# vganapati/CT_PVAE

Hardware: AMD Instinct MI355X
Metric: projections/sec (fwd+adj) 128x128 foam, 20 angles; fraction of HBM roofline (higher is better)
Workload: dtype f32; 1 GPU; batch=50/GPU 128x128 foam, 20 angles, P=184, rotate nearest fwd + tf_compat adj; objects_per_gpu=50, n_pixel=128, angles=20, num_proj_pix=184, parallelism=batch-shard x1, forward_plan=u16 taps, launch=19 replays of a HIP graph of 100 steps + 66 steps launched from Python

## Files before the change

ct_pvae_amd/_lib.py:

```python
import ctypes
import os

_HERE = os.path.dirname(os.path.abspath(__file__))
LIB_PATH = os.path.join(_HERE, "libctpvae_radon.so")

NEAREST, BILINEAR = 0, 1
NOISE = {"gaussian": 0, "poisson": 1}
BWD_TF_COMPAT, BWD_EXACT = 0, 1
SIDDON_STORE = {"raysum": 0, "sirt": 1, "tv_dual": 2, "gaussian": 3, "poisson": 4, "ratio": 5}
EINVAL, EHIP, ENODEV = -1, -2, -3
ABI_VERSION = 3400

_c_int, _c_float, _vp = ctypes.c_int, ctypes.c_float, ctypes.c_void_p
_ip = ctypes.POINTER(ctypes.c_int)

SIGNATURES = {
    "ctpvae_abi_version": (_c_int, []),
    "ctpvae_last_error": (ctypes.c_char_p, []),
    "ctpvae_device_count": (_c_int, []),
    "ctpvae_tune_set": (_c_int, [ctypes.c_char_p, _c_int]),
    "ctpvae_tune_active": (_c_int, []),
    "ctpvae_num_proj_pix": (_c_int, [_c_int, _c_int]),
    "ctpvae_pad_amounts": (_c_int, [_c_int, _c_int, _ip, _ip]),
    "ctpvae_rotate_transforms_f32": (_c_int, [_vp, _c_int, _c_int, _c_int, _vp, _vp, _vp]),
    "ctpvae_rotate_transforms_host_f32": (_c_int, [_vp, _c_int, _c_int, _c_int, _vp, _vp]),
    "ctpvae_rotate_fwd_planned_sel_f32": (_c_int, [_vp, _c_int, _c_int, _c_int, _c_int, _c_int, _c_int, _vp, _vp, _c_int, _vp, _vp]),
    "ctpvae_rotate_fwd_planned_loglik_sel_f32": (_c_int, [_vp, _c_int, _c_int, _c_int, _c_int, _c_int, _c_int, _vp, _vp, _c_int,
                                                          _vp, _vp, _c_int, _vp, _c_float, _vp, _vp, _vp, _vp]),
    "ctpvae_rotate_cplan_supported": (_c_int, [_c_int, _c_int, _c_int, _c_int, _c_int, _c_int]),
    "ctpvae_rotate_cplan_bytes": (ctypes.c_longlong, [_c_int, _c_int, _c_int, _c_int, _c_int]),
    "ctpvae_rotate_cplan_build_f32": (_c_int, [_vp, _c_int, _c_int, _c_int, _c_int, _c_int, _c_int, _c_int, _vp, _vp]),
    "ctpvae_rotate_cplan_overflowed": (_c_int, [_vp, _c_int, _c_int, _c_int, _c_int, _c_int, _vp]),
    "ctpvae_rotate_fwd_compact_f32": (_c_int, [_vp, _c_int, _c_int, _c_int, _c_int, _c_int, _c_int, _vp, _vp, _c_int, _c_int, _vp,
                                               _vp, _c_int, _vp, _c_float, _vp, _vp, _vp, _vp, _vp, _vp]),
    "ctpvae_rotate_fwd_compact_noise_f32": (_c_int, [_vp, _c_int, _c_int, _c_int, _c_int, _c_int, _c_int, _vp, _vp, _c_int, _c_int, _vp,
                                                     _vp, _c_int, _vp, _c_float, _c_int, _vp, _vp, _vp, _vp, _vp, _vp]),
    "ctpvae_loglik_tasks_per_row": (_c_int, [_c_int, _c_int]),
    "ctpvae_loglik_part_floats": (ctypes.c_longlong, [_c_int, _c_int, _c_int, _c_int]),
    "ctpvae_loglik_object_sums_f32": (_c_int, [_vp, _c_int, _c_int, _c_int, _c_int, _vp, _vp]),
    "ctpvae_rotate_bwd_sel_scaled_f32": (_c_int, [_vp, _c_int, _c_int, _c_int, _c_int, _vp, _vp, _c_int, _c_int, _c_int, _c_int,
                                                  _c_int, _vp, ctypes.c_longlong, _vp, _vp]),
    "ctpvae_rotate_bwd4_plan_bytes": (ctypes.c_longlong, [_c_int, _c_int, _c_int, _c_int, _c_int]),
    "ctpvae_rotate_bwd4_plan_build_f32": (_c_int, [_vp, _c_int, _c_int, _c_int, _c_int, _c_int, _c_int, _c_int, _vp, _vp]),
    "ctpvae_rotate_bwd_planned_sel_scaled_f32": (_c_int, [_vp, _c_int, _c_int, _c_int, _c_int, _c_int, _c_int, _vp, _vp, _c_int,
                                                          _c_int, _vp, ctypes.c_longlong, _vp, _vp]),
    "ctpvae_rotate_fwd_f32": (_c_int, [_vp, _c_int, _c_int, _c_int, _c_int, _c_int, _c_int, _c_int, _vp, _c_int,
                                       _c_int, _vp, _vp]),
    "ctpvae_rotate_fwd_f64": (_c_int, [_vp, _c_int, _c_int, _c_int, _c_int, _c_int, _c_int, _c_int, _vp, _c_int,
                                       _c_int, _vp, _vp]),
    "ctpvae_rotate_bwd_f64": (_c_int, [_vp, _c_int, _c_int, _c_int, _c_int, _vp, _c_int, _c_int, _c_int, _c_int,
                                       _c_int, _c_int, _vp, _vp]),
    "ctpvae_rotate_tile_shape": (_c_int, [_c_int, _c_int, _c_int, ctypes.POINTER(ctypes.c_int), ctypes.POINTER(ctypes.c_int)]),
    "ctpvae_rotate_fwd_tiled_workspace_bytes": (ctypes.c_longlong, [_c_int, _c_int, _c_int, _c_int, _c_int, _c_int, _c_int]),
    "ctpvae_rotate_fwd_tiled_f32": (_c_int, [_vp, _c_int, _c_int, _c_int, _c_int, _c_int, _c_int, _c_int, _vp, _c_int, _vp,
                                             _vp, _vp]),
    "ctpvae_rotate_fwd_tiled_interp_f32": (_c_int, [_vp, _c_int, _c_int, _c_int, _c_int, _c_int, _c_int, _c_int, _vp, _c_int, _c_int,
                                                    _vp, _vp, _vp]),
    "ctpvae_rotate_fwd_fast_f32": (_c_int, [_vp, _c_int, _c_int, _c_int, _c_int, _c_int, _c_int, _c_int, _vp, _c_int, _vp, _vp]),
    "ctpvae_rotate_fwd_tiled_fast_f32": (_c_int, [_vp, _c_int, _c_int, _c_int, _c_int, _c_int, _c_int, _c_int, _vp, _c_int, _vp,
                                                  _vp, _vp]),
    "ctpvae_rotate_fwd_tiled_loglik_f32": (_c_int, [_vp, _c_int, _c_int, _c_int, _c_int, _c_int, _c_int, _c_int, _vp, _c_int,
                                                    _vp, _vp, _vp, _vp, _c_float, _vp, _vp, _vp, _vp]),
    "ctpvae_rotate_tplan_bytes": (ctypes.c_longlong, [_c_int, _c_int, _c_int, _c_int, _c_int]),
    "ctpvae_rotate_tplan_build_f32": (_c_int, [_vp, _c_int, _c_int, _c_int, _c_int, _c_int, _c_int, _c_int, _vp, _vp]),
    "ctpvae_rotate_tplan_overflowed": (_c_int, [_vp, _c_int, _c_int, _c_int, _c_int, _c_int, _vp]),
    "ctpvae_rotate_fwd_tiled_compact_f32": (_c_int, [_vp, _c_int, _c_int, _c_int, _c_int, _c_int, _c_int, _c_int, _vp, _c_int, _vp,
                                                     _vp, _vp, _vp, _vp, _c_float, _vp, _vp, _vp, _vp, _vp, _vp]),
    "ctpvae_rotate_bwd_f32": (_c_int, [_vp, _c_int, _c_int, _c_int, _c_int, _vp, _c_int, _c_int, _c_int, _c_int,
                                       _c_int, _c_int, _vp, _vp]),
    "ctpvae_rotate_bwd_scaled_f32": (_c_int, [_vp, _c_int, _c_int, _c_int, _c_int, _vp, _c_int, _c_int, _c_int, _c_int,
                                              _c_int, _c_int, _vp, ctypes.c_longlong, _vp, _vp]),
    "ctpvae_rotate_plan_supported": (_c_int, [_c_int, _c_int, _c_int, _c_int, _c_int, _c_int, _c_int]),
    "ctpvae_rotate_plan_bytes": (ctypes.c_longlong, [_c_int, _c_int, _c_int, _c_int, _c_int, _c_int]),
    "ctpvae_rotate_plan_build_f32": (_c_int, [_vp, _vp, _c_int, _c_int, _c_int, _c_int, _c_int, _c_int, _c_int, _vp, _vp,
                                              _vp]),
    "ctpvae_rotate_fwd_planned_f32": (_c_int, [_vp, _c_int, _c_int, _c_int, _c_int, _c_int, _c_int, _vp, _vp, _vp]),
    "ctpvae_rotate_fwd_planned_form": (_c_int, [_c_int, _c_int, _c_int, _c_int, _c_int, _c_int, _c_int]),
    "ctpvae_rotate_fwd_planned_loglik_f32": (_c_int, [_vp, _c_int, _c_int, _c_int, _c_int, _c_int, _c_int, _vp, _vp, _vp, _vp,
                                                      _c_float, _vp, _vp, _vp, _vp]),
    "ctpvae_rotate_bwd_planned_f32": (_c_int, [_vp, _c_int, _c_int, _c_int, _c_int, _c_int, _c_int, _vp, _vp, _vp]),
    "ctpvae_rotate_bwd_planned_scaled_f32": (_c_int, [_vp, _c_int, _c_int, _c_int, _c_int, _c_int, _c_int, _vp, _vp,
                                                      ctypes.c_longlong, _vp, _vp]),
    "ctpvae_rotate_exact_plan_bytes": (ctypes.c_longlong, [_c_int, _c_int, _c_int, _c_int, _c_int]),
    "ctpvae_rotate_exact_plan_build_f32": (_c_int, [_vp, _vp, _c_int, _c_int, _c_int, _c_int, _c_int, _c_int, _c_int, _vp, _vp]),
    "ctpvae_rotate_exact_plan_overflowed": (_c_int, [_vp, _c_int, _c_int, _c_int, _c_int, _c_int, _vp]),
    "ctpvae_rotate_bwd_exact_planned_f32": (_c_int, [_vp, _c_int, _c_int, _c_int, _c_int, _c_int, _c_int, _vp, _vp, _vp]),
    "ctpvae_rotate_exact_wplan_bytes": (ctypes.c_longlong, [_c_int, _c_int, _c_int]),
    "ctpvae_rotate_exact_wplan_build_f32": (_c_int, [_vp, _vp, _c_int, _c_int, _c_int, _c_int, _c_int, _c_int, _c_int, _c_int, _vp, _vp]),
    "ctpvae_rotate_exact_wplan_overflowed": (_c_int, [_vp, _c_int, _c_int, _c_int, _vp]),
    "ctpvae_rotate_bwd_exact_wplan_f32": (_c_int, [_vp, _c_int, _c_int, _c_int, _c_int, _vp, _c_int, _c_int, _c_int, _c_int, _vp,
                                                              _vp, _vp]),
    "ctpvae_rotate_bwd_step_plan_bytes": (ctypes.c_longlong, [_c_int, _c_int, _c_int]),
    "ctpvae_rotate_bwd_step_plan_build_f32": (_c_int, [_vp, _c_int, _c_int, _c_int, _c_int, _c_int, _c_int, _c_int, _vp, _vp]),
    "ctpvae_rotate_bwd_step_plan_overflowed": (_c_int, [_vp, _c_int, _c_int, _c_int, _vp]),
    "ctpvae_rotate_bwd_stepped_scaled_f32": (_c_int, [_vp, _c_int, _c_int, _c_int, _c_int, _vp, _c_int, _c_int, _c_int, _c_int, _vp, _vp,
                                                      ctypes.c_longlong, _vp, _vp]),
    "ctpvae_siddon_dx": (_c_int, [_c_int, _c_int, _c_int]),
    "ctpvae_siddon_tables_f32": (_c_int, [_vp, _c_int, _vp, _vp, _vp]),
    "ctpvae_siddon_fwd_f32": (_c_int, [_vp, _c_int, _c_int, _c_int, _vp, _vp, _vp, _c_int, _c_int, _c_float, _vp,
                                       _vp]),
    "ctpvae_siddon_bwd_workspace_bytes": (ctypes.c_longlong, [_c_int, _c_int, _c_int, _c_int, _c_int]),
    "ctpvae_siddon_bwd_prepare_f32": (_c_int, [_c_int, _c_int, _vp, _vp, _vp, _c_int, _c_int, _c_float, _vp, _vp]),
    "ctpvae_siddon_bwd_prepared_f32": (_c_int, [_vp, _c_int, _c_int, _c_int, _vp, _vp, _vp, _c_int, _c_int, _c_float, _vp, _vp, _vp,
                                                _vp]),
    "ctpvae_siddon_fwd_workspace_bytes": (ctypes.c_longlong, [_c_int, _c_int, _c_int]),
    "ctpvae_siddon_fwd_ws_f32": (_c_int, [_vp, _c_int, _c_int, _c_int, _vp, _vp, _vp, _c_int, _c_int, _c_float, _vp, _vp, _vp, _vp,
                                          _vp]),
    "ctpvae_siddon_fwd_ws_tv_dual_f32": (_c_int, [_vp, _c_int, _c_int, _c_int, _vp, _vp, _vp, _c_int, _c_int, _c_float, _vp, _vp, _vp,
                                                  _vp, _vp]),
    "ctpvae_siddon_bwd_tv_primal_f32": (_c_int, [_vp, _c_int, _c_int, _c_int, _vp, _vp, _vp, _c_int, _c_int, _c_float, _vp, _vp,
                                                 _c_float, _vp, _vp, _vp, _vp, _vp, _vp, _vp, _vp]),
    "ctpvae_siddon_fwd_loglik_f32": (_c_int, [_vp, _c_int, _c_int, _c_int, _vp, _vp, _vp, _c_int, _c_int, _c_float, _vp, _c_int, _vp, _vp,
                                              _c_int, _vp, _c_float, _vp, _vp, _vp, _vp, _vp]),
    "ctpvae_siddon_fwd_loglik_noise_f32": (_c_int, [_vp, _c_int, _c_int, _c_int, _vp, _vp, _vp, _c_int, _c_int, _c_float, _vp, _c_int, _vp,
                                                    _vp, _c_int, _vp, _c_float, _c_int, _vp, _vp, _vp, _vp, _vp]),
    "ctpvae_siddon_bwd_sel_scaled_f32": (_c_int, [_vp, _c_int, _c_int, _c_int, _vp, _vp, _vp, _c_int, _c_int, _c_float, _vp, _c_int, _vp,
                                                  _vp, ctypes.c_longlong, _vp, _vp]),
    "ctpvae_siddon_fwd_ratio_f32": (_c_int, [_vp, _c_int, _c_int, _c_int, _vp, _vp, _vp, _c_int, _c_int, _c_float, _vp, _c_int, _vp, _vp,
                                             _vp, _vp]),
    "ctpvae_siddon_bwd_sel_mul_f32": (_c_int, [_vp, _c_int, _c_int, _c_int, _vp, _vp, _vp, _c_int, _c_int, _c_float, _vp, _c_int, _vp,
                                               _vp, _vp, _vp]),
    "ctpvae_siddon_bwd_sel_pml_f32": (_c_int, [_vp, _c_int, _c_int, _c_int, _vp, _vp, _vp, _c_int, _c_int, _c_float, _vp, _c_int, _vp,
                                               _vp, _c_float, _c_float, _c_int, _vp, _vp, _vp]),
    "ctpvae_siddon_fwd_resid_f32": (_c_int, [_vp, _c_int, _c_int, _c_int, _vp, _vp, _vp, _c_int, _c_int, _c_float, _vp, _vp, _vp,
                                             _vp]),
    "ctpvae_siddon_bwd_f32": (_c_int, [_vp, _c_int, _c_int, _c_int, _vp, _vp, _vp, _c_int, _c_int, _c_float, _vp, _vp, _vp]),
    "ctpvae_siddon_rownorm_f32": (_c_int, [_c_int, _c_int, _vp, _vp, _vp, _c_int, _c_int, _c_float, _vp, _vp]),
    "ctpvae_siddon_fwd_form": (_c_int, [_c_int, _c_int, _c_int, _c_int, _c_int, _c_int]),
    "ctpvae_fbp_filter_f64": (_c_int, [_vp, _c_int, _c_int, _vp, _vp, _vp]),
    "ctpvae_fbp_backproject_f64": (_c_int, [_vp, _c_int, _c_int, _c_int, _vp, _vp, _c_int, _c_int, _vp, _vp]),
    "ctpvae_fbp_backproject_bwd_f64": (_c_int, [_vp, _c_int, _c_int, _c_int, _vp, _vp, _c_int, _c_int, ctypes.c_double,
                                                ctypes.c_double, ctypes.c_double, _vp, _vp]),
    "ctpvae_fbp_backproject_geom_f64": (_c_int, [_vp, _c_int, _c_int, _c_int, _vp, _vp, _c_int, _c_int, ctypes.c_double,
                                                 ctypes.c_double, ctypes.c_double, _vp, _vp]),
    "ctpvae_gridrec_tables_bytes": (ctypes.c_longlong, [_c_int, _c_int]),
    "ctpvae_gridrec_tables_host_f32": (_c_int, [_c_int, _c_int, _c_float, _vp, _c_int, _vp, _vp]),
    "ctpvae_gridrec_workspace_bytes": (ctypes.c_longlong, [_c_int, _c_int, _c_int]),
    "ctpvae_gridrec_f32": (_c_int, [_vp, _c_int, _c_int, _c_int, _vp, _c_int, _c_int, _vp, _vp, _vp]),
    "ctpvae_poisson_loglik_fwd_f32": (_c_int, [_vp, _vp, _vp, _c_int, _c_int, _c_int, _vp, _vp, _vp]),
    "ctpvae_poisson_loglik_bwd_f32": (_c_int, [_vp, _vp, _vp, _vp, _c_int, _c_int, _c_int, _vp, _vp, _vp]),
    "ctpvae_loglik_fwd_f32": (_c_int, [_vp, _vp, _vp, _c_int, _c_int, _c_int, _vp, _c_float, _vp, _vp]),
    "ctpvae_poisson_measure_f32": (_c_int, [_vp, _vp, _c_int, _c_int, _c_int, _c_float, ctypes.c_ulonglong, _vp, _vp]),
    "ctpvae_philox4x32_10": (_c_int, [_vp, _vp, _vp]),
    "ctpvae_loglik_bwd_f32": (_c_int, [_vp, _vp, _vp, _vp, _c_int, _c_int, _c_int, _vp, _c_float, _vp, _vp, _vp]),
    "ctpvae_hmc_state_floats": (_c_int, [_c_int]),
    "ctpvae_hmc_init_f32": (_c_int, [_vp, _c_int, _c_int, _c_int, _vp, _vp, _c_int, _vp, _vp, _c_float, _c_int, _vp, _vp, _vp, _vp,
                                     _c_float, _vp]),
    "ctpvae_hmc_run_f32": (_c_int, [_vp, _c_int, ctypes.c_uint, _c_int, _c_int, _vp, _vp, _c_int, _vp, _vp, _c_float, _c_int, _vp, _vp,
                                    _vp, _c_int, _c_int, ctypes.c_uint, ctypes.c_uint, ctypes.c_ulonglong, _vp, _vp, _vp, _vp, _vp]),
    "ctpvae_tn_head_fwd_f32": (_c_int, [_vp, _vp, _c_int, _c_int, ctypes.c_longlong, ctypes.c_ulonglong, ctypes.c_uint, _vp, _vp, _vp, _vp,
                                        _vp]),
    "ctpvae_tn_head_bwd_f32": (_c_int, [_vp, _vp, _c_int, _c_int, ctypes.c_longlong, ctypes.c_ulonglong, ctypes.c_uint, _vp, _vp, _vp, _vp,
                                        _vp, _vp]),
    "ctpvae_tn_head_uniforms_host_f32": (_c_int, [_c_int, _c_int, ctypes.c_longlong, ctypes.c_ulonglong, ctypes.c_uint, _vp]),
    "ctpvae_tn_marginals_workspace_bytes": (ctypes.c_longlong, [_c_int, _c_int, ctypes.c_uint]),
    "ctpvae_tn_marginals_f32": (_c_int, [_vp, _vp, _c_int, _c_int, ctypes.c_longlong, ctypes.c_ulonglong, ctypes.c_uint, ctypes.c_uint,
                                         _c_float, _c_float, _c_int, _vp, _vp, _vp, _vp, _vp]),
    "ctpvae_tn_marginals_bin_host_f32": (_c_int, [_vp, ctypes.c_longlong, _c_float, _c_float, _c_int, _vp]),
    "ctpvae_latent_fwd_f32": (_c_int, [_vp, _c_int, _c_int, _c_int, _c_float, ctypes.c_longlong, ctypes.c_ulonglong, ctypes.c_uint,
                                       ctypes.c_uint, _vp, _vp, _vp, _vp, _vp, _vp]),
# ... 162 lines not shown
```

ct_pvae_amd/csrc/common.h:

```cpp
#pragma once
#include <hip/hip_runtime.h>
#include <atomic>
#include <cstdarg>
#include <cstdio>
#include <cstdlib>

#include "../../include/ctpvae_radon.h"

namespace ctpvae {

char *err_buf();
int fail(int code, const char *fmt, ...);

#define CTPVAE_REQUIRE(cond, ...)                                   \
    do {                                                            \
        if (!(cond)) return ::ctpvae::fail(CTPVAE_EINVAL, __VA_ARGS__); \
    } while (0)

#define CTPVAE_HIP(call)                                                                      \
    do {                                                                                      \
        hipError_t e_ = (call);                                                               \
        if (e_ != hipSuccess)                                                                 \
            return ::ctpvae::fail(CTPVAE_EHIP, "%s failed: %s", #call, hipGetErrorString(e_)); \
    } while (0)

#define CTPVAE_LAUNCH_CHECK(name)                                                             \
    do {                                                                                      \
        hipError_t e_ = hipGetLastError();                                                    \
        if (e_ != hipSuccess)                                                                 \
            return ::ctpvae::fail(CTPVAE_EHIP, "launch of %s failed: %s", name, hipGetErrorString(e_)); \
    } while (0)

constexpr int kMaxLdsBytes = 160 * 1024;

struct SliceScale {
    const float *ptr;
    long long stride;
    __device__ __forceinline__ float at(int s) const { return ptr ? ptr[(long long)s * stride] : 1.0f; }
};

enum StorePolicy { kStorePlain = 0, kStoreWriteThrough = 1, kStoreNonTemporal = 2 };
template <int ST> __device__ __forceinline__ void store_f32(float v, float *p)
{
    if constexpr (ST == kStoreWriteThrough) __hip_atomic_store(p, v, __ATOMIC_RELAXED, __HIP_MEMORY_SCOPE_AGENT);
    else if constexpr (ST == kStoreNonTemporal) __builtin_nontemporal_store(v, p);
    else *p = v;
}
template <int ST> __device__ __forceinline__ void store_f32x2(float v0, float v1, float *p)
{
    typedef float f2_t __attribute__((ext_vector_type(2)));
    const f2_t v = {v0, v1};
    if constexpr (ST == kStoreWriteThrough)
        __hip_atomic_store(reinterpret_cast<unsigned long long *>(p), __builtin_bit_cast(unsigned long long, v), __ATOMIC_RELAXED,
                           __HIP_MEMORY_SCOPE_AGENT);
    else if constexpr (ST == kStoreNonTemporal) __builtin_nontemporal_store(v, reinterpret_cast<f2_t *>(p));
    else *reinterpret_cast<f2_t *>(p) = v;
}

#define CTPVAE_SET_MAX_LDS_ONCE(kernel, seen)                                                                     \
    do {                                                                                                          \
        int dev_ = 0;                                                                                             \
        CTPVAE_HIP(hipGetDevice(&dev_));                                                                          \
        const unsigned long long bit_ = 1ull << (dev_ & 63);                                                      \
        if (dev_ >= 64 || !((seen).load(std::memory_order_acquire) & bit_)) {                                     \
            CTPVAE_HIP(hipFuncSetAttribute((const void *)(kernel), hipFuncAttributeMaxDynamicSharedMemorySize,    \
                                           ::ctpvae::kMaxLdsBytes));                                              \
            if (dev_ < 64) (seen).fetch_or(bit_, std::memory_order_release);                                      \
        }                                                                                                         \
    } while (0)

#define CTPVAE_REQUIRE_NO_STATIC_LDS(kernel, name, seen)                                                           \
    do {                                                                                                          \
        int dev_ = 0;                                                                                             \
        CTPVAE_HIP(hipGetDevice(&dev_));                                                                          \
        const unsigned long long bit_ = 1ull << (dev_ & 63);                                                      \
        const int fake_ = ::ctpvae::knob(::ctpvae::kKnobFakeStaticLds);                                            \
        if (dev_ >= 64 || fake_ > 0 || !((seen).load(std::memory_order_acquire) & bit_)) {                        \
            hipFuncAttributes fa_;                                                                                \
            CTPVAE_HIP(hipFuncGetAttributes(&fa_, (const void *)(kernel)));                                       \
            const long long static_ = (long long)fa_.sharedSizeBytes + (fake_ > 0 ? fake_ : 0);                    \
            if (static_ != 0)                                                                                     \
                return ::ctpvae::fail(CTPVAE_EHIP, "%s was built with %lld bytes of static LDS: its gathers address LDS " \
                                      "absolutely and need the dynamic array at address 0 -- rebuild the library (no "    \
                                      "__shared__ variables in these kernels)", name, static_);                   \
            if (dev_ < 64 && fake_ <= 0) (seen).fetch_or(bit_, std::memory_order_release);                        \
        }                                                                                                         \
    } while (0)

enum Knob {
    kKnobNoPlan, kKnobForceGeneric, kKnobNs, kKnobG, kKnobWaves, kKnobBns, kKnobBw, kKnobSegNs, kKnobSegChunk,
    kKnobSegPpt, kKnobTiledNs, kKnobTiledG, kKnobSiddonNs, kKnobSiddonThreads, kKnobSiddonPpb, kKnobMaxSlices,
    kKnobSiddonBwdNs, kKnobSiddonBwdChunks, kKnobNoCompact, kKnobSkew0, kKnobTiledSort, kKnobTiledPair, kKnobAffine, kKnobFakeStaticLds, kKnobFoldSums, kKnobTiledXcd, kKnobTiledWaves, kKnobTiledTh, kKnobReduceWaves, kKnobStepNs, kKnobStepLdsKb, kKnobTiledForce, kKnobBsort, kKnobMixG, kKnobMixG2, kKnobMixU1, kKnobNoMagic, kKnobMixG1, kKnobMixG3, kKnobMixU2, kKnobBrsplit, kKnobFwdFew, kKnobWtStores, kKnobBwdTail, kKnobCount
};
int knob(Knob k);

inline int store_policy(int rule)
{
    const int v = knob(kKnobWtStores);
    return v >= 0 && v <= 2 ? v : rule;
}

inline int max_slices_per_launch()
{
    const int v = knob(kKnobMaxSlices);
    return (v >= 1 && v <= 65535) ? v : 65535;
}

inline int ceil_div(int a, int b) { return (a + b - 1) / b; }

}
```

ct_pvae_amd/csrc/core.hip:

```cpp
#include <cmath>
#include <cstring>

#include "common.h"

namespace ctpvae {

char *err_buf()
{
    static thread_local char buf[512] = {0};
    return buf;
}

int fail(int code, const char *fmt, ...)
{
    va_list ap;
    va_start(ap, fmt);
    vsnprintf(err_buf(), 512, fmt, ap);
    va_end(ap);
    return code;
}

static const char *const kKnobNames[kKnobCount] = {
    "NO_PLAN", "FORCE_GENERIC", "NS", "G", "WAVES", "BNS", "BW", "SEG_NS", "SEG_CHUNK", "SEG_PPT", "TILED_NS", "TILED_G",
    "SIDDON_NS", "SIDDON_THREADS", "SIDDON_PPB", "MAX_SLICES", "SIDDON_BWD_NS", "SIDDON_BWD_CHUNKS", "NO_COMPACT", "SKEW0", "TILED_SORT", "TILED_PAIR", "AFFINE", "FAKE_STATIC_LDS", "FOLD_SUMS", "TILED_XCD", "TILED_WAVES", "TILED_TH", "REDUCE_WAVES", "STEP_NS", "STEP_LDS_KB", "TILED_FORCE", "BSORT", "MIXG", "MIXG_G2", "MIXG_U1", "NO_MAGIC", "MIXG_G1", "MIXG_G3", "MIXG_U2", "BRSPLIT", "FWD_FEW", "WT_STORES", "BWD_TAIL"};
static std::atomic<int> g_knobs[kKnobCount];
static int find_knob(const char *name)
{
    for (int k = 0; k < kKnobCount; ++k)
        if (strcmp(name, kKnobNames[k]) == 0) return k;
    return -1;
}
static const bool g_knobs_loaded = [] {
    for (int k = 0; k < kKnobCount; ++k) {
        int v = -1;
        char env[64];
        if (k == kKnobNoPlan || k == kKnobForceGeneric) {
            snprintf(env, sizeof env, "CTPVAE_%s", kKnobNames[k]);
            if (getenv(env) != nullptr) v = 1;
        } else {
            snprintf(env, sizeof env, "CTPVAE_TUNE_%s", kKnobNames[k]);
            if (const char *e = getenv(env)) v = atoi(e);
        }
        g_knobs[k].store(v, std::memory_order_relaxed);
    }
    return true;
}();
int knob(Knob k) { return g_knobs[k].load(std::memory_order_relaxed); }

__host__ __device__ static void inv3x3(const float m[9], float out[9])
{
    float a[3][6];
#pragma unroll
    for (int r = 0; r < 3; ++r)
#pragma unroll
        for (int c = 0; c < 3; ++c) {
            a[r][c] = m[3 * r + c];
            a[r][3 + c] = (r == c) ? 1.0f : 0.0f;
        }
#pragma unroll
    for (int k = 0; k < 3; ++k) {
        int p = k;
        for (int r = k + 1; r < 3; ++r)
            if (fabsf(a[r][k]) > fabsf(a[p][k])) p = r;
        if (p != k)
            for (int c = 0; c < 6; ++c) {
                float t = a[k][c];
                a[k][c] = a[p][c];
                a[p][c] = t;
            }
        for (int r = k + 1; r < 3; ++r) {
            const float f = a[r][k] / a[k][k];
            for (int c = k; c < 6; ++c) a[r][c] = a[r][c] - f * a[k][c];
        }
    }
    for (int c = 3; c < 6; ++c)
        for (int r = 2; r >= 0; --r) {
            float v = a[r][c];
            for (int q = r + 1; q < 3; ++q) v = v - a[r][q] * a[q][c];
            a[r][c] = v / a[r][r];
        }
    for (int r = 0; r < 3; ++r)
        for (int c = 0; c < 3; ++c) out[3 * r + c] = a[r][3 + c];
}

__host__ __device__ static void transform_rows(float theta, float hm1, float wm1, float *t8, float *tinv8)
{
    const float ang = -theta;
    const float c = (float)cos((double)ang);
    const float s = (float)sin((double)ang);
    const float cw = c * wm1, sh = s * hm1, sw = s * wm1, ch = c * hm1;
    const float xo = (wm1 - (cw - sh)) / 2.0f;
    const float yo = (hm1 - (sw + ch)) / 2.0f;
    const float t[8] = {c, -s, xo, s, c, yo, 0.0f, 0.0f};
    for (int k = 0; k < 8; ++k) t8[k] = t[k];
    if (tinv8) {
        const float m[9] = {t[0], t[1], t[2], t[3], t[4], t[5], t[6], t[7], 1.0f};
        float inv[9];
        inv3x3(m, inv);
        for (int k = 0; k < 8; ++k) tinv8[k] = inv[k] / inv[8];
    }
}

__global__ void rotate_transforms_kernel(const float *__restrict__ theta, int A, float hm1, float wm1,
                                         float *__restrict__ T8, float *__restrict__ Tinv8)
{
    const int a = blockIdx.x * blockDim.x + threadIdx.x;
    if (a >= A) return;
// ... 81 lines not shown
```

ct_pvae_amd/csrc/lds_stage.h:

```cpp
#pragma once
#include <hip/hip_runtime.h>
#include <cstdint>

namespace ctpvae {

__device__ __forceinline__ void stage_rows_v4(float *lds, const float *__restrict__ src, int rows, int cols, int src_stride,
                                              int pitch, bool mirror, int lane, int wave, int nwaves, int es = 1)
{
    const int ncb = (cols + 31) >> 5, npc = (ncb + 1) >> 1, nrq = (rows + 3) >> 2;
    const int npairs = nrq * npc;
    const int h = lane >> 5, k = (lane & 31) >> 3, m = lane & 7;
    constexpr int NB = 8;
    const int d_rq = nwaves / npc, d_pc = nwaves - d_rq * npc;
    int rq = wave / npc, pc = wave - rq * npc;
    for (int p0 = wave; p0 < npairs; p0 += NB * nwaves) {
        float4 v[NB];
        int r_[NB], c_[NB];
#pragma unroll
        for (int u = 0; u < NB; ++u) {
            r_[u] = 4 * rq + k;
            c_[u] = 32 * (2 * pc + h) + 4 * m;
            const bool ok = rq < nrq && r_[u] < rows && c_[u] < cols;
            const int rl = min(r_[u], rows - 1), cl = min(c_[u], cols - 4);
            v[u] = *reinterpret_cast<const float4 *>(src + (size_t)rl * src_stride + (mirror ? cols - 4 - cl : cl));
// ... 106 lines not shown
            const bool ok = rq < nrq && r_[u] < rows && c_[u] < cols;
            const int rl = min(r_[u], rows - 1), cl = min(c_[u], cols - 4);
#pragma unroll
            for (int n = 0; n < NS; ++n) v[u][n] = *reinterpret_cast<const float4 *>(src[n] + (size_t)rl * src_stride + cl);
            if (!ok) r_[u] = -1;
        }
    }
    __device__ __forceinline__ void commit(float *lds, int pitch) const
    {
        typedef float vec_t __attribute__((ext_vector_type(NS)));
#pragma unroll
        for (int u = 0; u < NB; ++u) {
            if (r_[u] < 0) continue;
            vec_t *d = reinterpret_cast<vec_t *>(lds) + (r_[u] * pitch + c_[u]);
            vec_t w0, w1, w2, w3;
#pragma unroll
            for (int n = 0; n < NS; ++n) {
                w0[n] = v[u][n].x;
                w1[n] = v[u][n].y;
                w2[n] = v[u][n].z;
                w3[n] = v[u][n].w;
            }
            d[0] = w0;
            d[1] = w1;
            d[2] = w2;
            d[3] = w3;
        }
    }
};

template <int NS, int NB, bool MIRROR, class F>
__device__ __forceinline__ void stage_unit_pow2_m(float *lds, const float *const (&src)[NS], int rows, int cs, int src_stride, int pitch,
                                                  int lane, int wave, int nwaves, F between)
{
    const int h = lane >> 5, k = (lane & 31) >> 3, m = lane & 7, cols = 64 << cs, nrq = rows >> 2;
    const int lo_src = k * src_stride + (MIRROR ? -(32 * h + 4 * m) : 32 * h + 4 * m);
    const int lo_dst = k * pitch + 32 * h + 4 * m;
    float4 v[NB][NS];
#pragma unroll
    for (int i = 0; i < NB; ++i) {
        const int pp = wave + i * nwaves, rq = pp >> cs, pc = pp & ((1 << cs) - 1);
        const int so = rq < nrq ? 4 * rq * src_stride + (MIRROR ? cols - 4 - 64 * pc : 64 * pc) : (MIRROR ? cols - 4 : 0);
#pragma unroll
        for (int n = 0; n < NS; ++n) v[i][n] = *reinterpret_cast<const float4 *>(src[n] + so + lo_src);
    }
    between();
#pragma unroll
    for (int i = 0; i < NB; ++i) {
        const int pp = wave + i * nwaves, rq = pp >> cs, pc = pp & ((1 << cs) - 1);
        if (rq >= nrq) continue;
        const int cell = 4 * rq * pitch + 64 * pc + lo_dst;
        if constexpr (NS == 1) {
            float *d = lds + cell;
            d[0] = MIRROR ? v[i][0].w : v[i][0].x;
            d[1] = MIRROR ? v[i][0].z : v[i][0].y;
            d[2] = MIRROR ? v[i][0].y : v[i][0].z;
            d[3] = MIRROR ? v[i][0].x : v[i][0].w;
        } else {
            typedef float vec_t __attribute__((ext_vector_type(NS)));
            vec_t *d = reinterpret_cast<vec_t *>(lds) + cell;
            vec_t w0, w1, w2, w3;
#pragma unroll
            for (int n = 0; n < NS; ++n) {
                w0[n] = MIRROR ? v[i][n].w : v[i][n].x;
                w1[n] = MIRROR ? v[i][n].z : v[i][n].y;
                w2[n] = MIRROR ? v[i][n].y : v[i][n].z;
                w3[n] = MIRROR ? v[i][n].x : v[i][n].w;
            }
            d[0] = w0;
            d[1] = w1;
            d[2] = w2;
            d[3] = w3;
        }
    }
}
template <int NS, int NB, class F>
__device__ __forceinline__ void stage_unit_pow2(float *lds, const float *const (&src)[NS], int rows, int cs, int src_stride, int pitch,
                                                bool mirror, int lane, int wave, int nwaves, F between)
{
    if (mirror) stage_unit_pow2_m<NS, NB, true>(lds, src, rows, cs, src_stride, pitch, lane, wave, nwaves, between);
    else stage_unit_pow2_m<NS, NB, false>(lds, src, rows, cs, src_stride, pitch, lane, wave, nwaves, between);
}

__host__ __device__ inline int contig_rows_units_per_quad(int cols) { return (cols + 15) >> 4; }
__host__ __device__ inline unsigned contig_rows_magic(int cols) { return 65536u / (unsigned)contig_rows_units_per_quad(cols) + 1u; }
__host__ __device__ inline int contig_rows_units(int rows, int cols) { return ((rows + 3) >> 2) * contig_rows_units_per_quad(cols); }
template <int NS, int NB, class F>
__device__ __forceinline__ void stage_contig_rows_batch(float *lds, const float *const (&src)[NS], int rows, int cols, int pitch,
                                                        unsigned magic, int tid, int nthreads, int u0, F between)
{
    typedef float vec_t __attribute__((ext_vector_type(NS)));
    const unsigned c4 = (unsigned)cols >> 2, upr = (unsigned)contig_rows_units_per_quad(cols);
    const int nunits = contig_rows_units(rows, cols), ngroups = nthreads >> 4;
    const unsigned grp = (unsigned)tid >> 4, k = ((unsigned)tid >> 2) & 3u, m = (unsigned)tid & 3u;
    float4 v[NB][NS];
    int cell[NB];
#pragma unroll
    for (int i = 0; i < NB; ++i) {
        if (u0 + i * ngroups >= nunits) continue;
        const unsigned U = (unsigned)(u0 + i * ngroups) + grp;
        const unsigned rq = __umul24(U, magic) >> 16, uc = U - __umul24(rq, upr);
        const unsigned row = 4u * rq + k, col4 = 4u * uc + m;
        const bool ok = row < (unsigned)rows && col4 < c4;
        const unsigned off = ok ? (__umul24(row, c4) + col4) << 4 : 0u;
        cell[i] = ok ? (int)(__umul24(row, (unsigned)pitch) + 4u * col4) : -1;
#pragma unroll
        for (int n = 0; n < NS; ++n) v[i][n] = *reinterpret_cast<const float4 *>(reinterpret_cast<const char *>(src[n]) + off);
    }
    between();
#pragma unroll
    for (int i = 0; i < NB; ++i) {
        if (u0 + i * ngroups >= nunits || cell[i] < 0) continue;
        vec_t *d = reinterpret_cast<vec_t *>(lds) + cell[i];
        vec_t w0, w1, w2, w3;
#pragma unroll
        for (int n = 0; n < NS; ++n) {
            w0[n] = v[i][n].x;
            w1[n] = v[i][n].y;
            w2[n] = v[i][n].z;
            w3[n] = v[i][n].w;
        }
        d[0] = w0;
        d[1] = w1;
        d[2] = w2;
        d[3] = w3;
    }
}
template <int NS, int NB, class F>
__device__ __forceinline__ void stage_contig_rows(float *lds, const float *const (&src)[NS], int rows, int cols, int pitch, unsigned magic,
                                                  int tid, int nthreads, F between)
{
    stage_contig_rows_batch<NS, NB>(lds, src, rows, cols, pitch, magic, tid, nthreads, 0, between);
}
template <int NB> __device__ __forceinline__ bool contig_rows_more(int rows, int cols, int nthreads)
{
    return contig_rows_units(rows, cols) > NB * (nthreads >> 4);
}
template <int NS, int NB>
__device__ __forceinline__ void stage_contig_rows_rest(float *lds, const float *const (&src)[NS], int rows, int cols, int pitch,
                                                       unsigned magic, int tid, int nthreads)
{
    const int step = NB * (nthreads >> 4);
    for (int u0 = step; u0 < contig_rows_units(rows, cols); u0 += step)
        stage_contig_rows_batch<NS, NB>(lds, src, rows, cols, pitch, magic, tid, nthreads, u0, [] {});
}

__device__ __forceinline__ int unit_pow2_cs(int rows, int cols, int src_stride, int nwaves, int nb)
{
#ifdef CTPVAE_TUNE_NO_LEAN_STAGE
    return -1;
#else
    if ((rows & 3) != 0 || (src_stride & 3) != 0 || (cols != 64 && cols != 128 && cols != 256)) return -1;
    const int cs = cols == 64 ? 0 : (cols == 128 ? 1 : 2);
    return ((rows >> 2) << cs) <= nb * nwaves ? cs : -1;
#endif
}
__device__ __forceinline__ void stage_rows(float *lds, const float *__restrict__ src, int rows, int cols, int src_stride,
                                           int pitch, bool mirror, int lane, int wave, int nwaves, int es = 1)
{
    if ((cols & 3) == 0 && (src_stride & 3) == 0 && (reinterpret_cast<uintptr_t>(src) & 15) == 0)
        stage_rows_v4(lds, src, rows, cols, src_stride, pitch, mirror, lane, wave, nwaves, es);
    else
        stage_rows_scalar(lds, src, rows, cols, src_stride, pitch, mirror, wave * 64 + lane, nwaves * 64, es);
}

template <int NS>
// ... 34 lines not shown
```

ct_pvae_amd/csrc/rotate_plan.hip:

```cpp
#include <algorithm>
#include <atomic>
#include <climits>
#include <cstdlib>
#include <type_traits>

#include "common.h"
#include "lds_stage.h"
#include "loglik_math.h"
#include "rotate_plan.h"
#include "tune_stamps.h"

namespace ctpvae {

struct FwdLayout {
    int nJB, PWpad, NG, Galloc, pitch, zero, skew0;
    long long off_cls, off_clist, off_first, off_rng, off_idx, bytes;
};
constexpr int kBwdPitch = 257;
constexpr int kBwdChunk = 64;
struct BwdLayout {
    int nXB, Wpad, NA16, pitchg, chunkA;
    long long bytes;
};

static FwdLayout fwd_layout(const PlanGeom &g)
{
    FwdLayout L;
    L.nJB = num_bin_blocks(g.PW);
    L.PWpad = L.nJB * 64;
    L.NG = ceil_div(g.PH, 8);
    L.Galloc = L.NG + 8;
    L.skew0 = knob(kKnobSkew0) > 0 ? 1 : 0;
    L.pitch = L.skew0 ? (g.W + 31) / 32 * 32 : pitch_mod32_is_1(g.W);
    if (L.skew0) L.Galloc += 6;
    L.zero = g.H * L.pitch;
    L.off_cls = 0;
    L.off_clist = (long long)g.A * 4;
    L.off_first = (L.off_clist + 2ll * (g.A + 1) * 4 + 8 + 255) / 256 * 256;
    L.off_rng = (L.off_first + (long long)g.A * L.PWpad * 4 + 255) / 256 * 256;
    L.off_idx = (L.off_rng + (long long)g.A * L.nJB * 8 + 255) / 256 * 256;
    L.bytes = L.off_idx + (long long)g.A * L.Galloc * L.PWpad * 16;
    return L;
}
static int bwd_tail_dwords(int A, int dup)
{
    const int r = A % 16;
    return dup == 1 && r >= 1 && r <= 12 ? (r + 3) / 4 : 0;
}
static BwdLayout bwd_layout(const PlanGeom &g, int dup = 1)
{
    BwdLayout L;
    L.nXB = ceil_div(g.W, 64);
    L.Wpad = L.nXB * 64;
    L.NA16 = ceil_div(g.A * dup, 16);
    L.pitchg = kBwdPitch;
    L.chunkA = std::min(L.NA16 * 16, kBwdChunk);
    L.bytes = (long long)L.NA16 * g.H * L.Wpad * 16;
    L.bytes = (L.bytes + 255) / 256 * 256 + (long long)bwd_tail_dwords(g.A, dup) * g.H * L.Wpad * 4;
    return L;
}
static bool fwd_plan_fits(const PlanGeom &g)
{
    const FwdLayout L = fwd_layout(g);
    return L.zero < 65535 && (size_t)(L.zero + 1) * 4 + 16 <= (size_t)kMaxLdsBytes;
}
static bool bwd_plan_fits(const PlanGeom &g) { return g.PW <= 255; }

__device__ __forceinline__ int fwd_tap(const PlanGeom &g, const FwdLayout &L, bool plus, float xj, float yj, float t1,
                                       float t2, float t4, float t5, int i)
{
    const float fi = (float)i;
    const float x = (xj + t1 * fi) + t2;
    const float y = (yj + t4 * fi) + t5;
    const int ix = (int)__builtin_roundf(x) - g.px;
    const int iy = (int)__builtin_roundf(y) - g.py;
    if ((unsigned)ix < (unsigned)g.W && (unsigned)iy < (unsigned)g.H) return iy * L.pitch + (plus ? ix : g.W - 1 - ix);
    return -1;
}
__global__ __launch_bounds__(64) void rotate_fwd_first_kernel(PlanGeom g, const float *__restrict__ T8, FwdLayout L,
                                                              char *__restrict__ plan)
{
    const int a = blockIdx.y, jb = blockIdx.x, lane = threadIdx.x;
    const int j = lane_to_bin(g.PW, jb, lane);
    const float *t = T8 + 8 * a;
    const float t0 = t[0], t1 = t[1], t2 = t[2], t3 = t[3], t4 = t[4], t5 = t[5];
    const bool plus = L.skew0 ? true : (t0 >= 0.0f) == (t3 >= 0.0f);
    int *cls = reinterpret_cast<int *>(plan + L.off_cls);
    int *first = reinterpret_cast<int *>(plan + L.off_first);
    if (jb == 0 && lane == 0) cls[a] = L.skew0 ? (a & 1) : (plus ? 1 : 0);
    const float xj = t0 * (float)j, yj = t3 * (float)j;
    int f = g.PH;
    if ((unsigned)j < (unsigned)g.PW)
        for (int i = 0; i < g.PH; ++i)
            if (fwd_tap(g, L, plus, xj, yj, t1, t2, t4, t5, i) >= 0) {
                f = i;
                break;
            }
    if (L.skew0) {
        int best_steps = INT_MAX, best_start = f;
        for (int sgn = 0; sgn < 2; ++sgn) {
            const float target = sgn ? -1.0f : 1.0f;
            const float alpha = fabsf(t1) < 1e-3f ? 0.0f : (target - t0) / t1;
            const int d = (int)rintf(alpha * (float)(lane & 31));
            int cmin = f < g.PH ? f - d : INT_MAX;
            for (int off = 16; off > 0; off >>= 1) cmin = min(cmin, __shfl_xor(cmin, off, 64));
            const int start = cmin == INT_MAX ? f : d + cmin;
            int last = -1;
            if (f < g.PH)
                for (int i = g.PH - 1; i >= f; --i)
                    if (fwd_tap(g, L, plus, xj, yj, t1, t2, t4, t5, i) >= 0) {
                        last = i;
                        break;
                    }
            int steps = f < g.PH ? last - start + 1 : 0;
            for (int off = 32; off > 0; off >>= 1) steps = max(steps, __shfl_xor(steps, off, 64));
            if (steps < best_steps) {
                best_steps = steps;
                best_start = start;
            }
        }
        f = f < g.PH ? max(best_start, -(1 << 20)) : f;
    }
    first[(size_t)a * L.PWpad + jb * 64 + lane] = f;
}
constexpr int kRngBias = 0x7f7f7f7f;
__global__ __launch_bounds__(64) void rotate_fwd_plan_kernel(PlanGeom g, const float *__restrict__ T8, FwdLayout L,
                                                             char *__restrict__ plan)
{
    const int a = blockIdx.y, jb = blockIdx.x, gq = blockIdx.z, lane = threadIdx.x;
    const int j = lane_to_bin(g.PW, jb, lane);
    const float *t = T8 + 8 * a;
    const float t0 = t[0], t1 = t[1], t2 = t[2], t3 = t[3], t4 = t[4], t5 = t[5];
    const bool plus = L.skew0 ? true : (t0 >= 0.0f) == (t3 >= 0.0f);
    const int *first = reinterpret_cast<const int *>(plan + L.off_first);
    int *rng = reinterpret_cast<int *>(plan + L.off_rng);
    uint4 *idx = reinterpret_cast<uint4 *>(plan + L.off_idx);
    const float xj = t0 * (float)j, yj = t3 * (float)j;
    const int i0 = first[(size_t)a * L.PWpad + jb * 64 + lane] + 8 * gq;
    unsigned e16[8];
    bool any = false;
#pragma unroll
    for (int e = 0; e < 8; ++e) {
        const int i = i0 + e;
        unsigned v = (unsigned)L.zero;
        if (i >= 0 && i < g.PH && (unsigned)j < (unsigned)g.PW) {
            const int tap = fwd_tap(g, L, plus, xj, yj, t1, t2, t4, t5, i);
            if (tap >= 0) {
                v = (unsigned)tap;
                any = true;
            }
        }
        e16[e] = v;
    }
    uint4 q;
    q.x = e16[0] | (e16[1] << 16);
    q.y = e16[2] | (e16[3] << 16);
    q.z = e16[4] | (e16[5] << 16);
    q.w = e16[6] | (e16[7] << 16);
    idx[((size_t)a * L.Galloc + gq) * L.PWpad + jb * 64 + lane] = q;
    if (__any(any) && lane == 0) {
        atomicMin(&rng[(a * L.nJB + jb) * 2 + 0], gq);
        atomicMin(&rng[(a * L.nJB + jb) * 2 + 1], kRngBias - gq);
    }
}

__global__ __launch_bounds__(64) void rotate_bwd_plan_kernel(PlanGeom g, const float *__restrict__ Tinv8, BwdLayout L,
                                                             uint4 *__restrict__ idx, int tail_t)
{
    const int xb = blockIdx.x, yrow = blockIdx.y, a16 = blockIdx.z, lane = threadIdx.x;
    const int xcol = xb * 64 + lane;
    const float fx = (float)(xcol + g.px), fy = (float)(yrow + g.py);
    unsigned w[4] = {0u, 0u, 0u, 0u};
#pragma unroll
    for (int e = 0; e < 16; ++e) {
        const int a = 16 * a16 + e;
        unsigned v = 255u;
        if (a < g.A && xcol < g.W) {
            const float *t = Tinv8 + 8 * a;
            const float x = (t[0] * fx + t[1] * fy) + t[2];
            const float y = (t[3] * fx + t[4] * fy) + t[5];
            const int ix = (int)__builtin_roundf(x), iy = (int)__builtin_roundf(y);
            if ((unsigned)ix < (unsigned)g.PW && (unsigned)iy < (unsigned)g.PH) v = (unsigned)ix;
        }
        w[e >> 2] |= v << (8 * (e & 3));
    }
    idx[((size_t)a16 * g.H + yrow) * L.Wpad + xcol] = make_uint4(w[0], w[1], w[2], w[3]);
    if (tail_t > 0 && a16 == L.NA16 - 1) {
        unsigned *rec = reinterpret_cast<unsigned *>(idx + (size_t)L.NA16 * g.H * L.Wpad) + ((size_t)yrow * L.Wpad + xcol) * tail_t;
#pragma unroll
        for (int d = 0; d < 3; ++d)
            if (d < tail_t) rec[d] = w[d];
    }
}

__global__ __launch_bounds__(64) void rotate_exact_plan_kernel(PlanGeom g, const float *__restrict__ T8,
                                                               const float *__restrict__ Tinv8, BwdLayout L,
                                                               unsigned char *__restrict__ idx, int *__restrict__ overflow)
{
    const int xb = blockIdx.x, yrow = blockIdx.y, a = blockIdx.z, lane = threadIdx.x;
    const int xcol = xb * 64 + lane;
    unsigned hit0 = 255u, hit1 = 255u;
    if (xcol < g.W) {
        const float *ti = Tinv8 + 8 * a, *t = T8 + 8 * a;
        const float fx = (float)(xcol + g.px), fy = (float)(yrow + g.py);
        const int jc = (int)__builtin_roundf((ti[0] * fx + ti[1] * fy) + ti[2]);
        const int ic = (int)__builtin_roundf((ti[3] * fx + ti[4] * fy) + ti[5]);
        int n = 0;
        for (int i = ic - 1; i <= ic + 1; ++i)
            for (int j = jc - 1; j <= jc + 1; ++j) {
                if ((unsigned)i >= (unsigned)g.PH || (unsigned)j >= (unsigned)g.PW) continue;
                const float x = (t[0] * (float)j + t[1] * (float)i) + t[2];
                const float y = (t[3] * (float)j + t[4] * (float)i) + t[5];
                if ((int)__builtin_roundf(x) - g.px == xcol && (int)__builtin_roundf(y) - g.py == yrow) {
                    if (n == 0) hit0 = (unsigned)j;
                    if (n == 1) hit1 = (unsigned)j;
                    ++n;
                }
            }
        if (n > 2) atomicOr(overflow, 1);
    }
    unsigned char *cell = idx + (((size_t)((2 * a) >> 4) * g.H + yrow) * L.Wpad + xcol) * 16 + ((2 * a) & 15);
    cell[0] = (unsigned char)hit0;
    cell[1] = (unsigned char)hit1;
}

__device__ __forceinline__ void unpack2(unsigned pk, int &lo4, int &hi4)
{
    asm("v_lshlrev_b32_sdwa %0, 2, %1 dst_sel:DWORD dst_unused:UNUSED_PAD src0_sel:DWORD src1_sel:WORD_0"
        : "=v"(lo4)
        : "v"(pk));
    asm("v_lshlrev_b32_sdwa %0, 2, %1 dst_sel:DWORD dst_unused:UNUSED_PAD src0_sel:DWORD src1_sel:WORD_1"
        : "=v"(hi4)
        : "v"(pk));
}
__device__ __forceinline__ float lds_at(const float *, int byte_off) { return *(lds_cptr)(size_t)(unsigned)byte_off; }
__device__ __forceinline__ void unpack2x8(unsigned pk, int &lo8, int &hi8)
{
    asm("v_lshlrev_b32_sdwa %0, 3, %1 dst_sel:DWORD dst_unused:UNUSED_PAD src0_sel:DWORD src1_sel:WORD_0"
        : "=v"(lo8)
        : "v"(pk));
    asm("v_lshlrev_b32_sdwa %0, 3, %1 dst_sel:DWORD dst_unused:UNUSED_PAD src0_sel:DWORD src1_sel:WORD_1"
        : "=v"(hi8)
        : "v"(pk));
}
__device__ __forceinline__ void gather8(const float *lds, const uint4 q, f32x2 (&v)[8])
{
    int a[8];
    unpack2x8(q.x, a[0], a[1]);
    unpack2x8(q.y, a[2], a[3]);
    unpack2x8(q.z, a[4], a[5]);
    unpack2x8(q.w, a[6], a[7]);
#pragma unroll
    for (int e = 0; e < 8; ++e) v[e] = *(const __attribute__((address_space(3))) f32x2 *)(size_t)(unsigned)a[e];
}
__device__ __forceinline__ void gather8(const float *lds, const uint4 q, float (&v)[8])
{
    int a0, a1, a2, a3, a4, a5, a6, a7;
    unpack2(q.x, a0, a1);
    unpack2(q.y, a2, a3);
    unpack2(q.z, a4, a5);
    unpack2(q.w, a6, a7);
    v[0] = lds_at(lds, a0);
    v[1] = lds_at(lds, a1);
    v[2] = lds_at(lds, a2);
    v[3] = lds_at(lds, a3);
    v[4] = lds_at(lds, a4);
    v[5] = lds_at(lds, a5);
    v[6] = lds_at(lds, a6);
    v[7] = lds_at(lds, a7);
}

__host__ __device__ inline unsigned div_magic(unsigned d) { return d > 1 ? (unsigned)((1ull << 32) / d) + 1u : 0u; }
__host__ __device__ inline unsigned div_by_magic(unsigned x, unsigned magic) { return magic ? (unsigned)(((unsigned long long)x * magic) >> 32) : x; }
__host__ __device__ inline unsigned div_magic_floor(unsigned d) { return d > 1 ? (unsigned)((1ull << 32) / d) : 0xffffffffu; }
__host__ __device__ inline unsigned div_by_magic_floor(unsigned x, unsigned magic, unsigned d)
{
    const unsigned q = (unsigned)(((unsigned long long)x * magic) >> 32);
    return q + (x - q * d >= d ? 1u : 0u);
}

__global__ __launch_bounds__(64) void rotate_class_list_kernel(int A, FwdLayout L, char *__restrict__ plan)
{
    const int *cls = reinterpret_cast<const int *>(plan + L.off_cls);
    int *clist = reinterpret_cast<int *>(plan + L.off_clist);
    const int lane = threadIdx.x;
    for (int c = 0; c < 2; ++c) {
        int *list = clist + c * (A + 1);
        int n = 0;
        for (int a0 = 0; a0 < A; a0 += 64) {
            const bool in = a0 + lane < A && cls[a0 + lane] == c;
            const unsigned long long m = __ballot(in);
            if (in) list[1 + n + __popcll(m & ((1ull << lane) - 1ull))] = a0 + lane;
            n += __popcll(m);
        }
        if (lane == 0) {
            list[0] = n;
            reinterpret_cast<unsigned *>(clist + 2 * (A + 1))[c] = div_magic((unsigned)n);
        }
    }
}

constexpr int kSelRounds = 4;
#define CTPVAE_PADD(VC) _Pragma("unroll") for (int e = 0; e < 8; ++e) acc += VC[e];
#define CTPVAE_PSTEP(QN, VN, VC, LOADNEXT)    \
                gather8(lds, QN, VN);                                                              \
                LOADNEXT;                                                                          \
                __builtin_amdgcn_sched_barrier(0);                                                 \
                CTPVAE_PADD(VC)
#define CTPVAE_FWD_WALK_U16                                                                        \
            int n = 0;                                                                             \
            for (; n + 4 < ng; n += 4) {    \
                CTPVAE_PSTEP(q1, vb, va, q1 = p[st])                             \
                CTPVAE_PSTEP(q2, va, vb, q2 = p[2 * st])                          \
                CTPVAE_PSTEP(q3, vb, va, q3 = p[3 * st])                          \
                CTPVAE_PSTEP(q0, va, vb, (p += 4 * st, q0 = p[0]))                \
            }                                                                                      \
            if (n + 1 >= ng) {    \
                CTPVAE_PADD(va)                                                                    \
            } else {                                                                               \
                CTPVAE_PSTEP(q1, vb, va, (void)0)                                                  \
                if (n + 2 >= ng) {                                                                 \
                    CTPVAE_PADD(vb)                                                                \
                } else {                                                                           \
                    CTPVAE_PSTEP(q2, va, vb, (void)0)                                              \
                    if (n + 3 >= ng) {                                                             \
                        CTPVAE_PADD(va)                                                            \
                    } else {                                                                       \
                        CTPVAE_PSTEP(q3, vb, va, (void)0)                                          \
                        CTPVAE_PADD(vb)                                                            \
                    }                                                                              \
                }                                                                                  \
            }
template <int NS, bool EPI, bool SEL>
__global__ __launch_bounds__(1024) void rotate_fwd_planned_kernel(const float *__restrict__ img, PlanGeom g, FwdLayout L,
                                                                  const char *__restrict__ plan, int wgs_per_slice,
                                                                  int g_S, float *__restrict__ sino, LogLikEpilogue epi,
                                                                  const int *__restrict__ sel, int n_sel, int affine,
                                                                  int units1, int wgs2, unsigned inv_wgs1, unsigned inv_wgs2, int small_div,
                                                                  int units2, int wgs3, unsigned inv_wgs3)
{
    typedef typename SliceVec<NS>::type vec_t;
    extern __shared__ float lds[];
    const int units = (g_S + NS - 1) / NS;
    auto piece_of = [&](int q, int &u_, int &wg_, int &wgs_) {
        int u0 = 0, nu = units1;
        unsigned inv = inv_wgs1;
        wgs_ = wgs_per_slice;
        const int Q1 = units1 * wgs_per_slice, Q2 = (units2 - units1) * wgs2;
        if (q >= Q1 + Q2) {
            q -= Q1 + Q2;
            u0 = units2;
            nu = units - units2;
            wgs_ = wgs3;
            inv = inv_wgs3;
        } else if (q >= Q1) {
            q -= Q1;
            u0 = units1;
            nu = units2 - units1;
            wgs_ = wgs2;
            inv = inv_wgs2;
        }
        const int octet = small_div ? (int)div_by_magic((unsigned)q >> 3, inv) : q / (8 * wgs_), rem = q - octet * 8 * wgs_;
        if ((octet + 1) * 8 <= nu) {
            wg_ = rem >> 3;
            u_ = u0 + octet * 8 + (rem & 7);
        } else {
            const int ru = small_div ? (int)div_by_magic((unsigned)rem, inv) : rem / wgs_;
            u_ = u0 + octet * 8 + ru;
            wg_ = rem - ru * wgs_;
        }
    };
    int u, wg, wgs = wgs_per_slice;
    [[maybe_unused]] const int q = blockIdx.x;
    if (affine) {
        u = blockIdx.x / wgs_per_slice;
        wg = blockIdx.x - u * wgs_per_slice;
    } else {
        piece_of(q, u, wg, wgs);
    }
    const int s = u * NS;
    const bool has2 = NS == 2 && s + 1 < g_S;
    const int c = wg & 1, gi = wg >> 1, G = wgs >> 1;
    const int lane = threadIdx.x & 63, wave = threadIdx.x >> 6, nwaves = blockDim.x >> 6;
    const float *im = img + (size_t)s * g.H * g.W;
    CTPVAE_PSTAMP(0);

    const int *clist = reinterpret_cast<const int *>(plan + L.off_clist) + c * (g.A + 1);
    const int *rng = reinterpret_cast<const int *>(plan + L.off_rng);
    const uint4 *idx = reinterpret_cast<const uint4 *>(plan + L.off_idx);
    const int A_out = SEL ? n_sel : g.A;
    int sel_a[kSelRounds], sel_rank[kSelRounds], sel_cum[kSelRounds + 1];
    int ncls;
    if constexpr (SEL) {
        const int *cls = reinterpret_cast<const int *>(plan + L.off_cls);
        sel_cum[0] = 0;
#pragma unroll
        for (int r = 0; r < kSelRounds; ++r) {
            const int k = 64 * r + lane;
            int a = 0, cl = -1;
            if (k < n_sel) {
                a = min(max(sel[k], 0), g.A - 1);
                cl = cls[a];
            }
            const unsigned long long m = __ballot(cl == c);
            sel_a[r] = a;
            sel_rank[r] = cl == c ? (int)__popcll(m & ((1ull << lane) - 1ull)) : -1;
            sel_cum[r + 1] = sel_cum[r] + (int)__popcll(m);
        }
        ncls = sel_cum[kSelRounds];
    } else {
        ncls = clist[0];
    }
    [[maybe_unused]] const unsigned inv_ncls = reinterpret_cast<const unsigned *>(plan + L.off_clist + 2ll * (g.A + 1) * 4)[c];
    const int n_gi = affine ? max(0, (ncls - gi + G - 1) / G) : 0;
    const int ntask = affine ? n_gi * L.nJB : ncls * L.nJB;
// ... 32 lines not shown
            if constexpr (SEL) {
#pragma unroll
                for (int r = 0; r < kSelRounds; ++r)
                    if (ai >= sel_cum[r] && ai < sel_cum[r + 1]) {
                        const unsigned long long hit = __ballot(sel_rank[r] == ai - sel_cum[r]);
                        const int l = __builtin_amdgcn_readfirstlane((int)__ffsll((long long)hit) - 1);
                        t.a = __builtin_amdgcn_readlane(sel_a[r], l);
                        t.k = 64 * r + l;
                    }
            } else {
                t.k = t.a = clist[1 + ai];
            }
            const int first = rng[(t.a * L.nJB + jb) * 2], last = kRngBias - rng[(t.a * L.nJB + jb) * 2 + 1];
            const int g0 = last >= first ? first : 0;
            t.ng = last >= first ? last - first + 1 : 0;
            t.j = lane_to_bin(g.PW, jb, lane);
            t.p = idx + ((size_t)t.a * L.Galloc + g0) * L.PWpad + jb * 64 + lane;
            t.q0 = t.p[0];
            t.q1 = t.p[st];
            t.q2 = t.p[2 * st];
            t.q3 = t.p[3 * st];
            t.p += 4 * st;
            if constexpr (EPI) {
                const int jc = min(max(t.j, 0), g.PW - 1);
#pragma unroll
                for (int n = 0; n < NS; ++n) {
                    const int sl = min(s + n, g_S - 1);
                    const size_t sa = SEL && epi.dense ? (size_t)sl * g.A + t.a : (size_t)sl * A_out + t.k;
                    t.em[n] = epi.mask[sa];
                    t.ex[n] = epi.meas[sa * g.PW + jc];
                }
            }
        }
        return t;
    };
    Task cur = prepare(wave);
    int *next_task = reinterpret_cast<int *>(lds + (L.zero + 1) * NS);
    if (threadIdx.x == 0) *next_task = nwaves;

    {
        const float *srcs[NS];
        srcs[0] = im;
        if constexpr (NS == 2) srcs[1] = im + (has2 ? (size_t)g.H * g.W : 0);
        stage_unit<NS>(lds, srcs, g.H, g.W, g.W, L.pitch, c == 0 && !L.skew0, lane, wave, nwaves);
    }
    if (threadIdx.x < NS) lds[L.zero * NS + threadIdx.x] = 0.0f;
    CTPVAE_PSTAMP(1);
    __syncthreads();
    CTPVAE_PSTAMP(2);

    while (cur.valid) {
        int m = 0;
        if (lane == 0) m = atomicAdd(next_task, 1);
        const Task nxt = prepare(__builtin_amdgcn_readfirstlane(m));

        const int ng = __builtin_amdgcn_readfirstlane(cur.ng);
        const uint4 *p = cur.p;
        vec_t acc = 0.0f;
        if (ng > 0) {
            uint4 q0 = cur.q0, q1 = cur.q1, q2 = cur.q2, q3 = cur.q3;
            vec_t va[8], vb[8];
            gather8(lds, q0, va);
            q0 = p[0];
            CTPVAE_FWD_WALK_U16
        }
        if ((unsigned)cur.j < (unsigned)g.PW) {
            auto store = [&](int n, float v) {
                const size_t o = ((size_t)(s + n) * A_out + cur.k) * g.PW + cur.j;
                sino[o] = v;
                if constexpr (EPI) epi.write_loaded(o, cur.em[n], cur.ex[n], epnm, einv, v);
            };
            if constexpr (NS == 1) {
                store(0, acc);
            } else {
                store(0, acc.x);
                if (has2) store(1, acc.y);
            }
        }
        cur = nxt;
    }
    CTPVAE_PSTAMP(3);
}

struct FwdFewArgs {
    const int *clist;
    const unsigned *inv_ncls;
    const int *rng;
    const uint4 *idx;
    int A, A1, rows, cs, src_stride, pitch, zero, PW, nJB;
    int st, ast;
    int G, wgs, S, units, slice;
    unsigned inv_wgs;
};
template <int NS>
__global__ __launch_bounds__(1024) void rotate_fwd_planned_kernel_few(const float *__restrict__ img, float *__restrict__ sino, FwdFewArgs k)
{
    typedef typename SliceVec<NS>::type vec_t;
    extern __shared__ float lds[];
    const unsigned q = blockIdx.x, per8 = 8u * (unsigned)k.wgs;
    const unsigned octet = div_by_magic(q >> 3, k.inv_wgs), rem = q - octet * per8;
    int u, wg;
    if ((int)(octet + 1) * 8 <= k.units) {
        wg = rem >> 3;
        u = octet * 8 + (rem & 7);
    } else {
        const unsigned ru = div_by_magic(rem, k.inv_wgs);
        u = octet * 8 + ru;
        wg = rem - ru * k.wgs;
    }
    const int s = u * NS;
    const bool has2 = NS == 2 && s + 1 < k.S;
    const int c = wg & 1, gi = wg >> 1;
    const int lane = threadIdx.x & 63, nwaves = blockDim.x >> 6;
    const int wave = __builtin_amdgcn_readfirstlane(threadIdx.x >> 6);
    const float *im = img + (size_t)s * k.slice;
    CTPVAE_PSTAMP(0);

    const int *clist = k.clist + c * k.A1;
    const int ncls = clist[0], ntask = ncls * k.nJB;
    const unsigned inv_ncls = k.inv_ncls[c];
#ifdef CTPVAE_TUNE_NOIDX
    const size_t st = 0;
#else
    const size_t st = (size_t)k.st;
#endif
    struct Task {
        bool valid;
        int a, j, ng;
        const uint4 *p;
        uint4 q0, q1, q2, q3;
    };
    auto fill = [&](Task &t, int m) {
        const int jb = (int)div_by_magic((unsigned)m, inv_ncls), ai = m - jb * ncls;
        t.a = clist[1 + ai];
        const int first = k.rng[(t.a * k.nJB + jb) * 2], last = kRngBias - k.rng[(t.a * k.nJB + jb) * 2 + 1];
        const int g0 = last >= first ? first : 0;
        t.ng = last >= first ? last - first + 1 : 0;
        t.j = lane_to_bin(k.PW, jb, lane);
        t.p = k.idx + ((size_t)t.a * k.ast + (size_t)g0 * k.st + jb * 64) + lane;
        t.q0 = t.p[0];
        t.q1 = t.p[st];
        t.q2 = t.p[2 * st];
        t.q3 = t.p[3 * st];
        t.p += 4 * st;
    };
    Task cur;
    const int m0 = wave * k.G + gi;
    cur.valid = m0 < ntask;
    if (cur.valid) fill(cur, m0);
    int *next_task = reinterpret_cast<int *>(lds + (k.zero + 1) * NS);
    if (threadIdx.x == 0) *next_task = nwaves;

    {
        const float *srcs[NS];
        srcs[0] = im;
        if constexpr (NS == 2) srcs[1] = im + (has2 ? (size_t)k.slice : 0);
        if (c == 0) stage_unit_pow2_m<NS, 8 / NS, true>(lds, srcs, k.rows, k.cs, k.src_stride, k.pitch, lane, wave, nwaves, [] {});
        else stage_unit_pow2_m<NS, 8 / NS, false>(lds, srcs, k.rows, k.cs, k.src_stride, k.pitch, lane, wave, nwaves, [] {});
    }
    if (threadIdx.x < NS) lds[k.zero * NS + threadIdx.x] = 0.0f;
    CTPVAE_PSTAMP(1);
    __syncthreads();
    CTPVAE_PSTAMP(2);

    while (cur.valid) {
        int m = 0;
        if (lane == 0) m = atomicAdd(next_task, 1);
        Task nxt;
        {
            const int mn = __builtin_amdgcn_readfirstlane(m) * k.G + gi;
            nxt.valid = mn < ntask;
            if (nxt.valid) fill(nxt, mn);
        }
        const int ng = __builtin_amdgcn_readfirstlane(cur.ng);
        const uint4 *p = cur.p;
        vec_t acc = 0.0f;
        if (ng > 0) {
            uint4 q0 = cur.q0, q1 = cur.q1, q2 = cur.q2, q3 = cur.q3;
            vec_t va[8], vb[8];
            gather8(lds, q0, va);
            q0 = p[0];
            CTPVAE_FWD_WALK_U16
        }
        if ((unsigned)cur.j < (unsigned)k.PW) {
            const size_t o = ((size_t)s * k.A + cur.a) * k.PW + cur.j;
            if constexpr (NS == 1) {
                sino[o] = acc;
            } else {
                sino[o] = acc.x;
                if (has2) sino[o + (size_t)k.A * k.PW] = acc.y;
            }
        }
        cur = nxt;
    }
    CTPVAE_PSTAMP(3);
}
#undef CTPVAE_FWD_WALK_U16
#undef CTPVAE_PSTEP
#undef CTPVAE_PADD

template <int SHIFT>
__device__ __forceinline__ void unpack4(unsigned pk, int &b0, int &b1, int &b2, int &b3)
{
    asm("v_lshlrev_b32_sdwa %0, %2, %1 dst_sel:DWORD dst_unused:UNUSED_PAD src0_sel:DWORD src1_sel:BYTE_0" : "=v"(b0) : "v"(pk), "i"(SHIFT));
    asm("v_lshlrev_b32_sdwa %0, %2, %1 dst_sel:DWORD dst_unused:UNUSED_PAD src0_sel:DWORD src1_sel:BYTE_1" : "=v"(b1) : "v"(pk), "i"(SHIFT));
    asm("v_lshlrev_b32_sdwa %0, %2, %1 dst_sel:DWORD dst_unused:UNUSED_PAD src0_sel:DWORD src1_sel:BYTE_2" : "=v"(b2) : "v"(pk), "i"(SHIFT));
    asm("v_lshlrev_b32_sdwa %0, %2, %1 dst_sel:DWORD dst_unused:UNUSED_PAD src0_sel:DWORD src1_sel:BYTE_3" : "=v"(b3) : "v"(pk), "i"(SHIFT));
}
template <int NS> __device__ __forceinline__ typename SliceVec<NS>::type lds_at_vec(const float *, int byte_off)
{
    return *(const __attribute__((address_space(3))) typename SliceVec<NS>::type *)(size_t)(unsigned)byte_off;
}
template <int AL0, int T, int NS>
__device__ __forceinline__ void gather_dwords(const float *lds, const uint4 q, typename SliceVec<NS>::type (&v)[4 * T])
{
    static_assert(T >= 1 && T <= 4, "an index vector is four dwords");
    constexpr int ROW = kBwdPitch * 4 * NS;
    const unsigned w[4] = {q.x, q.y, q.z, q.w};
#pragma unroll
    for (int d = 0; d < T; ++d) {
        int b0, b1, b2, b3;
        unpack4<NS == 1 ? 2 : 3>(w[d], b0, b1, b2, b3);
        v[4 * d + 0] = lds_at_vec<NS>(lds, b0 + (AL0 + 4 * d + 0) * ROW);
        v[4 * d + 1] = lds_at_vec<NS>(lds, b1 + (AL0 + 4 * d + 1) * ROW);
        v[4 * d + 2] = lds_at_vec<NS>(lds, b2 + (AL0 + 4 * d + 2) * ROW);
        v[4 * d + 3] = lds_at_vec<NS>(lds, b3 + (AL0 + 4 * d + 3) * ROW);
    }
}

template <int AL0, int NS, int DUP = 1>
__device__ __forceinline__ void gather8(const float *lds, unsigned w0, unsigned w1, int n_live, typename SliceVec<NS>::type (&v)[8])
{
    constexpr int ROW = kBwdPitch * 4 * NS;
    const unsigned w[2] = {w0, w1};
#pragma unroll
    for (int d = 0; d < 2; ++d) {
        if (4 * d < n_live) {
            int b0, b1, b2, b3;
            unpack4<NS == 1 ? 2 : 3>(w[d], b0, b1, b2, b3);
            v[4 * d + 0] = lds_at_vec<NS>(lds, b0 + ((AL0 + 4 * d + 0) / DUP) * ROW);
            v[4 * d + 1] = lds_at_vec<NS>(lds, b1 + ((AL0 + 4 * d + 1) / DUP) * ROW);
            v[4 * d + 2] = lds_at_vec<NS>(lds, b2 + ((AL0 + 4 * d + 2) / DUP) * ROW);
            v[4 * d + 3] = lds_at_vec<NS>(lds, b3 + ((AL0 + 4 * d + 3) / DUP) * ROW);
        } else {
            v[4 * d + 0] = v[4 * d + 1] = v[4 * d + 2] = v[4 * d + 3] = 0.0f;
        }
    }
}

constexpr unsigned kIdxReqTail1 = 1u, kIdxReqTail2 = 2u, kIdxReqTail3 = 4u, kIdxReqFirst = 8u, kIdxReqTailWhole = 16u;
#define CTPVAE_BWD_PLANNED_KERNEL rotate_bwd_planned_kernel
#define CTPVAE_BWD_PLANNED_STORE kStorePlain
#include "rotate_bwd_planned_kernel.h"
#undef CTPVAE_BWD_PLANNED_KERNEL
#undef CTPVAE_BWD_PLANNED_STORE
#define CTPVAE_BWD_PLANNED_KERNEL rotate_bwd_planned_kernel_wt
#define CTPVAE_BWD_PLANNED_STORE kStoreWriteThrough
#include "rotate_bwd_planned_kernel.h"
#undef CTPVAE_BWD_PLANNED_KERNEL
#undef CTPVAE_BWD_PLANNED_STORE

__global__ __launch_bounds__(64) void rotate_bwd4_plan_kernel(PlanGeom g, const float *__restrict__ Tinv8, int Wpad, int HQ,
                                                              unsigned *__restrict__ idx4)
{
    const int xb = blockIdx.x, yq = blockIdx.y, a = blockIdx.z, lane = threadIdx.x;
    const int xcol = xb * 64 + lane;
    const float *t = Tinv8 + 8 * a;
    const float fx = (float)(xcol + g.px);
    unsigned w = 0u;
#pragma unroll
    for (int e = 0; e < 4; ++e) {
        const int yrow = 4 * yq + e;
        unsigned v = 255u;
        if (yrow < g.H && xcol < g.W) {
            const float fy = (float)(yrow + g.py);
            const float x = (t[0] * fx + t[1] * fy) + t[2];
            const float y = (t[3] * fx + t[4] * fy) + t[5];
            const int ix = (int)__builtin_roundf(x), iy = (int)__builtin_roundf(y);
            if ((unsigned)ix < (unsigned)g.PW && (unsigned)iy < (unsigned)g.PH) v = (unsigned)ix;
// ... 47 lines not shown
        for (int e = 0; e < 16; ++e) {
            const int k = min(kbase + e, n_sel - 1);
            const int a = min(max(HOSTSEL ? selh.get(k) : sel[k], 0), g.A - 1);
            q[e] = p[(size_t)a * astride];
        }
    };
    for (int kc = 0; kc < n_sel; kc += kChunk) {
        const int nk = min(kChunk, n_sel - kc);
        unsigned q0[16];
        load16(kc, q0);
        if (kc > 0) __syncthreads();
        for (int t = threadIdx.x; t < nk * NS; t += blockDim.x) lds[((t / NS) * kBwdPitch + 255) * NS + (t % NS)] = 0.0f;
        if constexpr (NS == 1) {
            stage_rows(lds, gs + (size_t)kc * g.PW, nk, g.PW, g.PW, kBwdPitch, false, lane, wave, nwaves);
        } else {
            const float *srcs[2] = {gs + (size_t)kc * g.PW, gs + (has2 ? (size_t)n_sel * g.PW : 0) + (size_t)kc * g.PW};
            stage_rows_interleaved<2>(lds, srcs, nk, g.PW, g.PW, kBwdPitch, false, lane, wave, nwaves);
        }
        auto block16 = [&](auto k0_tag) {
            constexpr int K0 = decltype(k0_tag)::value;
            if constexpr (K0 < kChunk) {
                if (K0 >= nk) return;
                unsigned q[16];
                if constexpr (K0 == 0) {
#pragma unroll
                    for (int e = 0; e < 16; ++e) q[e] = q0[e];
                    __syncthreads();
                } else {
                    load16(kc + K0, q);
                }
#pragma unroll
                for (int e = 0; e < 16; ++e) {
                    if (K0 + e < nk) {
                        int b0, b1, b2, b3;
                        unpack4<NS == 1 ? 2 : 3>(q[e], b0, b1, b2, b3);
                        acc[0] += lds_at_vec<NS>(lds, b0 + (K0 + e) * ROW);
                        acc[1] += lds_at_vec<NS>(lds, b1 + (K0 + e) * ROW);
                        acc[2] += lds_at_vec<NS>(lds, b2 + (K0 + e) * ROW);
                        acc[3] += lds_at_vec<NS>(lds, b3 + (K0 + e) * ROW);
                    }
                }
            }
        };
        block16(std::integral_constant<int, 0>{});
        block16(std::integral_constant<int, 16>{});
        block16(std::integral_constant<int, 32>{});
        block16(std::integral_constant<int, 48>{});
    }
    if (xcol < g.W && wave_live) {
#pragma unroll
        for (int e = 0; e < 4; ++e) {
            const int y = 4 * yq + e;
            if (y < g.H) {
                if constexpr (NS == 1) {
                    gimg[((size_t)s * g.H + y) * g.W + xcol] = k0 * acc[e];
                } else {
                    gimg[((size_t)s * g.H + y) * g.W + xcol] = k0 * acc[e].x;
                    if (has2) gimg[((size_t)(s + 1) * g.H + y) * g.W + xcol] = k1 * acc[e].y;
                }
            }
        }
    }
}

}

using namespace ctpvae;

extern "C" {

int ctpvae_rotate_plan_supported(int H, int W, int PH, int PW, int A, int interp, int which)
{
    if (interp != CTPVAE_NEAREST || H <= 0 || W <= 0 || PH < H || PW < W || A <= 0) return 0;
    if (knob(kKnobNoPlan) >= 0) return 0;
    if (which == 0 && knob(kKnobTiledForce) == 1) return 0;
    const PlanGeom g{H, W, PH, PW, 0, 0, A};
    return which == 0 ? (fwd_plan_fits(g) ? 1 : 0) : (bwd_plan_fits(g) ? 1 : 0);
}

long long ctpvae_rotate_plan_bytes(int H, int W, int PH, int PW, int A, int which)
{
    if (H <= 0 || W <= 0 || PH < H || PW < W || A <= 0) return fail(CTPVAE_EINVAL, "rotate_plan_bytes: bad sizes");
    const PlanGeom g{H, W, PH, PW, 0, 0, A};
    return which == 0 ? fwd_layout(g).bytes : bwd_layout(g).bytes;
}

int ctpvae_rotate_plan_build_f32(const float *T8_dev, const float *Tinv8_dev, int A, int H, int W, int PH, int PW, int py,
                                 int px, void *fwd_plan_dev, void *bwd_plan_dev, ctpvae_stream_t stream)
{
    if (int rc = check_plan_geom("rotate_plan_build", H, W, PH, PW, py, px, A)) return rc;
    CTPVAE_REQUIRE(fwd_plan_dev || bwd_plan_dev, "rotate_plan_build: no plan buffer given");
    const PlanGeom g{H, W, PH, PW, py, px, A};
    if (fwd_plan_dev) {
        CTPVAE_REQUIRE(T8_dev, "rotate_plan_build: forward plan needs the forward transforms");
        CTPVAE_REQUIRE(fwd_plan_fits(g), "rotate_plan_build: a %dx%d slice does not fit the forward plan's LDS image", H, W);
        CTPVAE_REQUIRE(A <= 65535, "rotate_plan_build: at most 65535 angles");
        const FwdLayout L = fwd_layout(g);
        CTPVAE_REQUIRE(L.Galloc <= 65535, "rotate_plan_build: canvas too tall");
        CTPVAE_HIP(hipMemsetAsync((char *)fwd_plan_dev + L.off_rng, 0x7f, (size_t)A * L.nJB * 8, (hipStream_t)stream));
        hipLaunchKernelGGL(rotate_fwd_first_kernel, dim3(L.nJB, A), dim3(64), 0, (hipStream_t)stream, g, T8_dev, L,
                           (char *)fwd_plan_dev);
        CTPVAE_LAUNCH_CHECK("rotate_fwd_first_kernel");
        hipLaunchKernelGGL(rotate_fwd_plan_kernel, dim3(L.nJB, A, L.Galloc), dim3(64), 0, (hipStream_t)stream, g, T8_dev, L,
                           (char *)fwd_plan_dev);
        CTPVAE_LAUNCH_CHECK("rotate_fwd_plan_kernel");
        hipLaunchKernelGGL(rotate_class_list_kernel, dim3(1), dim3(64), 0, (hipStream_t)stream, A, L, (char *)fwd_plan_dev);
        CTPVAE_LAUNCH_CHECK("rotate_class_list_kernel");
    }
    if (bwd_plan_dev) {
        CTPVAE_REQUIRE(Tinv8_dev, "rotate_plan_build: backward plan needs the inverted transforms");
        CTPVAE_REQUIRE(bwd_plan_fits(g), "rotate_plan_build: the backward plan stores bins as bytes (PW=%d > 255)", PW);
        CTPVAE_REQUIRE(H <= 65535, "rotate_plan_build: at most 65535 rows");
        const BwdLayout L = bwd_layout(g);
        hipLaunchKernelGGL(rotate_bwd_plan_kernel, dim3(L.nXB, H, L.NA16), dim3(64), 0, (hipStream_t)stream, g, Tinv8_dev, L,
                           (uint4 *)bwd_plan_dev, bwd_tail_dwords(A, 1));
        CTPVAE_LAUNCH_CHECK("rotate_bwd_plan_kernel");
    }
    return CTPVAE_OK;
}

constexpr double kRoundKb = 150.0;
static inline double launch_rounds(long long wgs)
{
    const double real = (double)wgs / 256.0, whole = std::ceil(real);
    return whole > 1.0 ? real + 0.75 * (whole - real) : 1.0;
}

struct FwdShape {
    PlanGeom g;
    FwdLayout L;
    int ns, affine, waves, units, wgs_per_slice, units1, wgs2, units2, wgs3, small_div;
    long long grid;
    size_t shmem;
};
static int fwd_planned_shape(int S, int H, int W, int PH, int PW, int A, bool has_sel, int n_sel, FwdShape &sh)
{
    CTPVAE_REQUIRE(S > 0, "rotate_fwd_planned: need at least one slice");
    if (int rc = check_plan_geom("rotate_fwd_planned", H, W, PH, PW, 0, 0, A)) return rc;
    CTPVAE_REQUIRE(!has_sel || (n_sel >= 1 && n_sel <= 64 * kSelRounds),
                   "rotate_fwd_planned: an angle subset holds 1..%d angles (got %d); build a plan for larger ones",
                   64 * kSelRounds, n_sel);
    const PlanGeom g{H, W, PH, PW, 0, 0, A};
    CTPVAE_REQUIRE(fwd_plan_fits(g), "rotate_fwd_planned: a %dx%d slice does not fit the plan's LDS image", H, W);
    const FwdLayout L = fwd_layout(g);
    const int A_run = has_sel ? n_sel : A;
    const int T = A_run * L.nJB;
    const bool pairs_fit = (size_t)(L.zero + 1) * 8 + 16 <= (size_t)kMaxLdsBytes && S >= 2;
    int ns = 1, G = 1, affine = 0;
    {
        const double task_kb = 0.6 * L.NG;
        const double plan_kb = (double)L.bytes * A_run / A / 1024.0;
        double best = 0.0, best_aff = 0.0;
        int ns_aff = 1, G_aff = 4;
        for (int cand_ns = 1; cand_ns <= (pairs_fit ? 2 : 1); ++cand_ns) {
            const double fill_kb = (double)g.H * g.W * 4.0 * cand_ns / 1024.0;
            const long long cand_units = (S + cand_ns - 1) / cand_ns;
            const double fabric_kb = 1.5 * plan_kb * (double)std::min<long long>(8, cand_units) / 256.0;
            for (int cand = 1; cand <= std::min(12, std::max(1, T / 2)); ++cand) {
                const long long wgs = 2ll * cand_units * cand;
                const double cost = launch_rounds(wgs) * (fill_kb + kRoundKb + task_kb * T / (2.0 * cand)) + fabric_kb;
                if (best == 0.0 || cost <= best * (wgs <= 256 ? 1.03 : 1.0)) {
                    best = best == 0.0 ? cost : std::min(best, cost);
                    ns = cand_ns;
                    G = cand;
                }
            }
            const double fabric_aff = 1.5 * (plan_kb / 8.0 + (double)cand_units * fill_kb * 8.0) / 256.0;
            for (int cand = 4; cand <= 12 && 2 * cand <= std::max(8, T) && cand_units <= 16; cand += 4) {
                const long long wgs = 2ll * cand_units * cand;
                const double cost = (double)((wgs + 255) / 256) * (fill_kb + task_kb * T / (2.0 * cand)) + fabric_aff;
                if (best_aff == 0.0 || cost <= best_aff * 1.03) {
                    best_aff = best_aff == 0.0 ? cost : std::min(best_aff, cost);
                    ns_aff = cand_ns;
                    G_aff = cand;
                }
            }
        }
        const bool can = !has_sel && T >= 8 && best_aff > 0.0;
        if (can && knob(kKnobAffine) != 0 && (knob(kKnobAffine) == 1 || (plan_kb > 3072.0 && best_aff < best))) {
            affine = 1;
            ns = ns_aff;
            G = G_aff;
        }
    }
    if (knob(kKnobNs) >= 0) {
        const int want = knob(kKnobNs) == 2 ? 2 : 1;
        if (want != ns) {
            ns = want;
            affine = 0;
            const double task_kb = 0.6 * L.NG, fill_kb = (double)g.H * g.W * 4.0 * ns / 1024.0;
// ... 75 lines not shown
        if (units1 < units && knob(kKnobMixG3) != 0) {
            auto launch3_us = [&](int c3, int u2) {
                struct Free { double t; long long n; } f[16] = {{0.0, 256}};
                int nf = 1;
                const long long cnt[3] = {2ll * units1 * G1, 2ll * (u2 - units1) * G2, 2ll * (units - u2) * c3};
                const double cost[3] = {piece_us(G1), piece_us(G2), piece_us(c3)};
                double end = 0.0;
                for (int part = 0; part < 3; ++part)
                    for (long long left = cnt[part]; left > 0;) {
                        int k = 0;
                        for (int i = 1; i < nf; ++i) if (f[i].t < f[k].t) k = i;
                        const long long n = std::min(left, f[k].n);
                        if (n < f[k].n && nf < 16) f[nf++] = {f[k].t, f[k].n - n}, f[k].n = n;
                        f[k].t += cost[part];
                        end = std::max(end, f[k].t);
                        left -= n;
                    }
                return end;
            };
            double best3 = launch3_us(G2, units);
            for (int c3 = G2 + 1; c3 <= std::min(gmax, G2 + 3); ++c3)
                for (int u2 = units1 + 4; u2 < units; u2 += 4) {
                    const double t = launch3_us(c3, u2);
                    if (t < best3 * 0.98) best3 = t, G3 = c3, units2 = u2;
                }
            if (G3 == G2) units2 = units;
        }
        cut_cache[cut_next++ % 8] = Cut{key, G1, G2, G3, units1, units2};
        }
        if (knob(kKnobMixG2) > 0 && knob(kKnobMixU1) >= 0)
            G1 = knob(kKnobMixG1) > 0 ? knob(kKnobMixG1) : G, G2 = knob(kKnobMixG2), units1 = std::min(units, knob(kKnobMixU1));
        wgs_per_slice = 2 * G1;
        wgs2 = 2 * G2, wgs3 = 2 * G3;
        if (knob(kKnobMixG2) > 0 && knob(kKnobMixU1) >= 0) wgs3 = wgs2, units2 = units;
        if (knob(kKnobMixG3) > 0 && knob(kKnobMixU2) >= 0)
            wgs3 = 2 * knob(kKnobMixG3), units2 = std::max(units1, std::min(units, knob(kKnobMixU2)));
        waves = std::min(16, std::max(stage_waves, (T + 2 * G1 - 1) / (2 * G1)));
        if (knob(kKnobWaves) > 0) waves = std::min(16, knob(kKnobWaves));
    }
    units2 = std::max(units1, std::min(units2, units));
    const long long grid = (long long)units1 * wgs_per_slice + (long long)(units2 - units1) * wgs2 + (long long)(units - units2) * wgs3;
    CTPVAE_REQUIRE(grid < (1ll << 31), "rotate_fwd_planned: too many slices");
#ifdef CTPVAE_TUNE_STAMPS
    g_pshape[1] = wgs_per_slice, g_pshape[2] = waves, g_pshape[5] = units1, g_pshape[6] = wgs2, g_pshape[7] = units2, g_pshape[8] = wgs3;
#endif
    const int small_div = (grid / 8 + 1) * (long long)std::max(wgs_per_slice, std::max(wgs2, wgs3)) < (1ll << 32) && (long long)A * L.nJB * A < (1ll << 32) &&
                                  knob(kKnobNoMagic) <= 0 ? 1 : 0;
    sh = FwdShape{g, L, ns, affine, waves, units, wgs_per_slice, units1, wgs2, units2, wgs3, small_div, grid, shmem};
    return CTPVAE_OK;
}

constexpr int kFewMaxTasks = 48;
static bool fwd_few_ok(const FwdShape &sh, bool dense, bool img_aligned16)
{
    if (knob(kKnobFwdFew) == 0) return false;
    const int H = sh.g.H, W = sh.g.W;
    const int tasks = ceil_div(sh.g.A * sh.L.nJB, sh.wgs_per_slice);
    if (knob(kKnobFwdFew) != 1 && tasks > kFewMaxTasks) return false;
    return dense && !sh.affine && sh.units1 == sh.units && sh.small_div && !sh.L.skew0 && (W == 64 || W == 128 || W == 256) && H % 4 == 0 &&
           (H / 4) * (W / 64) <= (8 / sh.ns) * sh.waves && img_aligned16;
}

static int launch_fwd_planned(const float *img_dev, int S, int H, int W, int PH, int PW, int A, const void *fwd_plan_dev,
                              float *sino_dev, const LogLikEpilogue &epi, const int *sel_dev, int n_sel,
                              ctpvae_stream_t stream)
{
    CTPVAE_REQUIRE(img_dev && fwd_plan_dev && sino_dev, "rotate_fwd_planned: null pointer");
    FwdShape sh;
    if (int rc = fwd_planned_shape(S, H, W, PH, PW, A, sel_dev != nullptr, n_sel, sh)) return rc;
    const PlanGeom &g = sh.g;
    const FwdLayout &L = sh.L;
    const int ns = sh.ns;
    if (fwd_few_ok(sh, !sel_dev && !epi.lp, (reinterpret_cast<uintptr_t>(img_dev) & 15) == 0)) {
        const char *plan = (const char *)fwd_plan_dev;
        FwdFewArgs k;
        k.clist = reinterpret_cast<const int *>(plan + L.off_clist);
        k.inv_ncls = reinterpret_cast<const unsigned *>(plan + L.off_clist + 2ll * (A + 1) * 4);
        k.rng = reinterpret_cast<const int *>(plan + L.off_rng);
        k.idx = reinterpret_cast<const uint4 *>(plan + L.off_idx);
        k.A = A, k.A1 = A + 1, k.rows = H, k.cs = W == 64 ? 0 : (W == 128 ? 1 : 2), k.src_stride = W, k.pitch = L.pitch, k.zero = L.zero;
        k.PW = PW, k.nJB = L.nJB, k.st = L.PWpad, k.ast = L.Galloc * L.PWpad;
        k.G = sh.wgs_per_slice / 2, k.wgs = sh.wgs_per_slice, k.S = S, k.units = sh.units, k.slice = H * W;
        k.inv_wgs = div_magic((unsigned)sh.wgs_per_slice);
        auto launch_few = [&](auto kernel) -> int {
            static std::atomic<unsigned long long> attr_set{0}, abs_ok{0};
            CTPVAE_REQUIRE_NO_STATIC_LDS(kernel, "rotate_fwd_planned_kernel_few", abs_ok);
            CTPVAE_SET_MAX_LDS_ONCE(kernel, attr_set);
            hipLaunchKernelGGL(kernel, dim3((unsigned)sh.grid), dim3(64 * sh.waves), sh.shmem, (hipStream_t)stream, img_dev, sino_dev, k);
            CTPVAE_LAUNCH_CHECK("rotate_fwd_planned_kernel_few");
            return CTPVAE_OK;
        };
        return ns == 2 ? launch_few(rotate_fwd_planned_kernel_few<2>) : launch_few(rotate_fwd_planned_kernel_few<1>);
    }
    auto launch = [&](auto kernel) -> int {
        static std::atomic<unsigned long long> attr_set{0}, abs_ok{0};
        CTPVAE_REQUIRE_NO_STATIC_LDS(kernel, "rotate_fwd_planned_kernel", abs_ok);
        CTPVAE_SET_MAX_LDS_ONCE(kernel, attr_set);
        hipLaunchKernelGGL(kernel, dim3((unsigned)sh.grid), dim3(64 * sh.waves), sh.shmem, (hipStream_t)stream,
                           img_dev, g, L, (const char *)fwd_plan_dev, sh.wgs_per_slice, S, sino_dev, epi, sel_dev, n_sel, sh.affine, sh.units1, sh.wgs2,
                           div_magic((unsigned)sh.wgs_per_slice), div_magic((unsigned)sh.wgs2), sh.small_div, sh.units2, sh.wgs3, div_magic((unsigned)sh.wgs3));
        CTPVAE_LAUNCH_CHECK("rotate_fwd_planned_kernel");
        return CTPVAE_OK;
    };
    if (sel_dev) {
        if (epi.lp) return ns == 2 ? launch(rotate_fwd_planned_kernel<2, true, true>) : launch(rotate_fwd_planned_kernel<1, true, true>);
        return ns == 2 ? launch(rotate_fwd_planned_kernel<2, false, true>) : launch(rotate_fwd_planned_kernel<1, false, true>);
    }
    if (epi.lp) return ns == 2 ? launch(rotate_fwd_planned_kernel<2, true, false>) : launch(rotate_fwd_planned_kernel<1, true, false>);
    return ns == 2 ? launch(rotate_fwd_planned_kernel<2, false, false>) : launch(rotate_fwd_planned_kernel<1, false, false>);
}

int ctpvae_rotate_fwd_planned_form(int S, int H, int W, int PH, int PW, int A, int img_aligned16)
{
    FwdShape sh;
    if (int rc = fwd_planned_shape(S, H, W, PH, PW, A, false, 0, sh)) return rc;
    return fwd_few_ok(sh, true, img_aligned16 != 0) ? 1 : 0;
}

int ctpvae_rotate_fwd_planned_f32(const float *img_dev, int S, int H, int W, int PH, int PW, int A, const void *fwd_plan_dev,
                                  float *sino_dev, ctpvae_stream_t stream)
{
    return launch_fwd_planned(img_dev, S, H, W, PH, PW, A, fwd_plan_dev, sino_dev, LogLikEpilogue{}, nullptr, 0, stream);
}

int ctpvae_rotate_fwd_planned_sel_f32(const float *img_dev, int S, int H, int W, int PH, int PW, int A,
                                      const void *fwd_plan_dev, const int *angle_idx_dev, int n_idx, float *sino_dev,
                                      ctpvae_stream_t stream)
{
    CTPVAE_REQUIRE(angle_idx_dev, "rotate_fwd_planned_sel: null angle index");
    return launch_fwd_planned(img_dev, S, H, W, PH, PW, A, fwd_plan_dev, sino_dev, LogLikEpilogue{}, angle_idx_dev, n_idx,
                              stream);
}

int ctpvae_rotate_fwd_planned_loglik_f32(const float *img_dev, int S, int H, int W, int PH, int PW, int A,
                                         const void *fwd_plan_dev, const float *mask_dev, const float *meas_dev,
                                         const float *pnm_dev, float eps, float *sino_dev, float *lp_dev,
                                         float *dlp_dev, ctpvae_stream_t stream)
{
    CTPVAE_REQUIRE(mask_dev && meas_dev && pnm_dev && lp_dev, "rotate_fwd_planned_loglik: null pointer");
    return launch_fwd_planned(img_dev, S, H, W, PH, PW, A, fwd_plan_dev, sino_dev,
                              LogLikEpilogue{mask_dev, meas_dev, pnm_dev, eps, lp_dev, dlp_dev, 0}, nullptr, 0, stream);
}

int ctpvae_rotate_fwd_planned_loglik_sel_f32(const float *img_dev, int S, int H, int W, int PH, int PW, int A,
                                             const void *fwd_plan_dev, const int *angle_idx_dev, int n_idx,
                                             const float *mask_dev, const float *meas_dev, int dense_inputs,
                                             const float *pnm_dev, float eps, float *sino_dev, float *lp_dev,
                                             float *dlp_dev, ctpvae_stream_t stream)
{
    CTPVAE_REQUIRE(angle_idx_dev && mask_dev && meas_dev && pnm_dev && lp_dev, "rotate_fwd_planned_loglik_sel: null pointer");
    return launch_fwd_planned(img_dev, S, H, W, PH, PW, A, fwd_plan_dev, sino_dev,
                              LogLikEpilogue{mask_dev, meas_dev, pnm_dev, eps, lp_dev, dlp_dev, dense_inputs ? 1 : 0},
                              angle_idx_dev, n_idx, stream);
}

int ctpvae_rotate_bwd_planned_f32(const float *gsino_dev, int S, int H, int W, int PH, int PW, int A, const void *bwd_plan_dev,
                                  float *gimg_dev, ctpvae_stream_t stream)
{
    return ctpvae_rotate_bwd_planned_scaled_f32(gsino_dev, S, H, W, PH, PW, A, bwd_plan_dev, nullptr, 0, gimg_dev, stream);
}

static int launch_bwd_planned(const float *gsino_dev, int S, int H, int W, int PH, int PW, int A, const void *bwd_plan_dev,
                              const float *scale_dev, long long scale_stride, float *gimg_dev, int dup,
                              ctpvae_stream_t stream)
{
    CTPVAE_REQUIRE(gsino_dev && bwd_plan_dev && gimg_dev, "rotate_bwd_planned: null pointer");
    CTPVAE_REQUIRE(S > 0, "rotate_bwd_planned: need at least one slice");
    if (int rc = check_plan_geom("rotate_bwd_planned", H, W, PH, PW, 0, 0, A)) return rc;
    const PlanGeom g{H, W, PH, PW, 0, 0, A};
    CTPVAE_REQUIRE(bwd_plan_fits(g), "rotate_bwd_planned: the backward plan stores bins as bytes (PW=%d > 255)", PW);
    const BwdLayout L = bwd_layout(g, dup);
    int ns = S >= 2 ? 2 : 1;
    const bool narrow = L.nXB == 1 && H > 32 && (long long)S * ceil_div(H, 16) < 512;
    if (narrow) ns = 1;
    if (knob(kKnobBns) >= 0) ns = (knob(kKnobBns) == 2 && S >= 2) ? 2 : 1;
    const int ppt = ns == 2 ? 2 : 4;
    const int units = ceil_div(S, ns);
    const size_t shmem = (size_t)std::min(ceil_div(L.NA16 * 16, dup), kBwdChunk / ns) * L.pitchg * sizeof(float) * ns;
    const int Aeff = A * dup;
    int waves = 4;
    if (ns == 2) {
        waves = Aeff >= 64 ? (S >= 32 ? 16 : 8) : (S > 16 ? 8 : 4);
        if (Aeff >= 32 && Aeff < 64 && waves == 8 && (long long)units * L.nXB * ceil_div(H, 8 * ppt) > 256 && (long long)units * L.nXB * ceil_div(H, 16 * ppt) <= 256)
            waves = 16;
        if (Aeff >= 64 && S >= 32) {
            auto wgs = [&](int w) { return (long long)units * L.nXB * ceil_div(H, w * ppt); };
            const int w_more = ceil_div(H, ppt * (ceil_div(H, 16 * ppt) + 1));
            if (wgs(8) <= 256)
                waves = 8;
            else if (w_more >= 9 && w_more < 16 && ceil_div((int)wgs(w_more), 256) == ceil_div((int)wgs(16), 256))
                waves = w_more;
        }
    }
    if (dup == 1 && A <= 32 && ns == 2 && S > 16) {
        auto wgs = [&](int w) { return (long long)units * L.nXB * ceil_div(H, w * ppt); };
        const long long r8 = (wgs(8) + 255) / 256, r11 = (wgs(11) + 255) / 256;
        if (r11 < r8 && r11 <= 2 && wgs(11) * 16 >= r11 * 256 * 15) waves = 11;
    }
    if (ns != 2 && Aeff >= 32 && !narrow)
// ... 181 lines not shown
```

ct_pvae_amd/forward_functions.py:

```python
import math
import os

import ctypes
import weakref

import numpy as np
import torch

from . import _lib

__all__ = ["pad_phantom", "project_tf_fast", "project_tf_low_mem", "num_proj_pix", "pad_amounts", "RotatePlan",
           "rotate_tables", "as_angle_index"]

_current_device = getattr(torch._C, "_cuda_getDevice", torch.cuda.current_device)
_INTERP = {"nearest": _lib.NEAREST, "bilinear": _lib.BILINEAR}
_BACKWARD = {"tf_compat": _lib.BWD_TF_COMPAT, "exact": _lib.BWD_EXACT}
_PRECISION = ("exact", "fast")


def _check_precision(precision, interp):
    if precision not in _PRECISION:
        raise ValueError(f"precision must be one of {list(_PRECISION)} (got {precision!r})")
    if precision == "fast" and interp != "bilinear":
        raise ValueError(f"precision='fast' needs interp='bilinear' (got interp={interp!r}): nearest has no weights to blend")
# ... 110 lines not shown
    MAX_SEL = 256
    COMPACT_MIN_ANGLES = 64
    COMPACT_DENSE_WINDOW = (36, 44)

    def __init__(self, theta, H, W, pad, device, interp="nearest", backward="tf_compat", use_plan=True, _tables=None,
                 plan_format="auto", precision="exact"):
        if plan_format not in ("auto", "compact", "u16"):
            raise ValueError(f"plan_format must be 'auto', 'compact' or 'u16' (got {plan_format!r})")
        if interp not in _INTERP:
            raise ValueError(f"interp must be one of {sorted(_INTERP)} (got {interp!r})")
        if backward not in _BACKWARD:
            raise ValueError(f"backward must be one of {sorted(_BACKWARD)} (got {backward!r})")
        _check_precision(precision, interp)
        self.precision, self.fast = precision, precision == "fast"
        self.H, self.W = int(H), int(W)
        if pad:
            P = num_proj_pix(self.H, self.W)
            self.PH = self.PW = P
            self.py, self.px = pad_amounts(self.H, P)[0], pad_amounts(self.W, P)[0]
        else:
            self.PH, self.PW, self.py, self.px = self.H, self.W, 0, 0
        self.device = torch.device(device)
        if self.device.type != "cuda":
            raise _lib.RadonLibraryError(
                f"the projector runs on a HIP device only (got a tensor on {self.device}); there is no CPU path")
        self.interp, self.mode = _INTERP[interp], _BACKWARD[backward]
        self._dev_index = self.device.index if self.device.index is not None else torch.cuda.current_device()
        self._interp_name, self._backward_name, self._pad = interp, backward, bool(pad)
        self.T8, self.Tinv8 = _tables if _tables is not None else rotate_tables(theta, self.PH, self.PW, self.device)
        self._tdev = self.T8.device
        self.A = self.T8.shape[0]
        self._lib = _lib.load()
        self._fwd_plan = self._bwd_plan = self._exact_plan = self._bwd4_plan = None
        self._want_bwd_plan = False
        self._want_bwd4 = bool(use_plan and self.interp == _lib.NEAREST and self.mode == _lib.BWD_TF_COMPAT)
        self._want_exact_plan = bool(use_plan and self.mode == _lib.BWD_EXACT and self.interp == _lib.NEAREST)
        self._use_tiles = bool(use_plan)
        self._tile_ws = None
        self._compact = False
        self._part_ws = {}
        self._u16_plan = None
        self._auto_dense_u16 = False
        if use_plan:
            geo = (self.H, self.W, self.PH, self.PW, self.A, self.interp)
            want_compact = plan_format == "compact" or (plan_format == "auto" and self.A >= self.COMPACT_MIN_ANGLES)
            if want_compact and self._lib.ctpvae_rotate_cplan_supported(*geo):
                self._fwd_plan = self._build_compact_plan()
                self._compact = self._fwd_plan is not None
            if self._fwd_plan is None and self._lib.ctpvae_rotate_plan_supported(*geo, 0):
                self._fwd_plan = self._build_plan(0)
            self._auto_dense_u16 = bool(plan_format == "auto" and self._compact and self._lib.ctpvae_rotate_plan_supported(*geo, 0))
            if self._auto_dense_u16:
                self._u16_plan = self._build_plan(0)
            self._want_bwd_plan = bool(self.mode == _lib.BWD_TF_COMPAT and
                                       self._lib.ctpvae_rotate_plan_supported(*geo, 1))
        self._tplan = None
        if (use_plan and self._fwd_plan is None and self.interp == _lib.NEAREST and plan_format != "u16"
                and self.py > 0 and self.px > 0):
            self._tplan = self._build_tile_plan()
        self._step_plan = None
        if (use_plan and self.interp == _lib.NEAREST and self.mode == _lib.BWD_TF_COMPAT and self.py > 0 and self.px > 0
                and self.A <= 65535 and self.H * self.W >= 128 * 128):
            self._step_plan = self._build_step_plan()
        self._exact_bilin_plan = None
        self._subsets = {}
        if use_plan and self.mode == _lib.BWD_EXACT:
            self._build_exact_plans()

    def _build_exact_plans(self):
        if self.interp == _lib.NEAREST:
            self._build_exact_plan()
        if self.H <= 65535 and (self.interp == _lib.BILINEAR or self._exact_plan is None):
            self._build_exact_bilinear_plan()

    def _build_plan(self, which):
        nbytes = self._lib.ctpvae_rotate_plan_bytes(self.H, self.W, self.PH, self.PW, self.A, which)
        _lib.check(nbytes, "rotate_plan_bytes")
        buf = torch.empty(int(nbytes), dtype=torch.uint8, device=self.device)
        with torch.cuda.device(self.device):
            _lib.check(self._lib.ctpvae_rotate_plan_build_f32(
                self.T8.data_ptr(), self.Tinv8.data_ptr(), self.A, self.H, self.W, self.PH, self.PW, self.py, self.px,
                buf.data_ptr() if which == 0 else None, buf.data_ptr() if which == 1 else None, _stream_ptr()),
                "rotate_plan_build")
        return buf

    def _build_compact_plan(self):
        nbytes = self._lib.ctpvae_rotate_cplan_bytes(self.H, self.W, self.PH, self.PW, self.A)
        _lib.check(nbytes, "rotate_cplan_bytes")
        buf = torch.empty(int(nbytes), dtype=torch.uint8, device=self.device)
        with torch.cuda.device(self.device):
            _lib.check(self._lib.ctpvae_rotate_cplan_build_f32(self.T8.data_ptr(), self.A, self.H, self.W, self.PH, self.PW,
                                                               self.py, self.px, buf.data_ptr(), _stream_ptr()),
                       "rotate_cplan_build")
            over = self._lib.ctpvae_rotate_cplan_overflowed(buf.data_ptr(), self.H, self.W, self.PH, self.PW, self.A,
                                                            _stream_ptr())
        _lib.check(over, "rotate_cplan_overflowed")
        return buf if over == 0 else None

    def _build_tile_plan(self):
        nbytes = self._lib.ctpvae_rotate_tplan_bytes(self.H, self.W, self.PH, self.PW, self.A)
        _lib.check(nbytes, "rotate_tplan_bytes")
        if nbytes == 0:
            return None
        buf = torch.empty(int(nbytes), dtype=torch.uint8, device=self.device)
        with torch.cuda.device(self.device):
            _lib.check(self._lib.ctpvae_rotate_tplan_build_f32(self.T8.data_ptr(), self.A, self.H, self.W, self.PH, self.PW, self.py,
                                                               self.px, buf.data_ptr(), _stream_ptr()), "rotate_tplan_build")
            over = self._lib.ctpvae_rotate_tplan_overflowed(buf.data_ptr(), self.H, self.W, self.PH, self.PW, self.A, _stream_ptr())
        _lib.check(over, "rotate_tplan_overflowed")
        return buf if over == 0 else None

    def _get_bwd4_plan(self):
        if self._bwd4_plan is None and self._want_bwd4:
            self._want_bwd4 = False
            nbytes = self._lib.ctpvae_rotate_bwd4_plan_bytes(self.H, self.W, self.PH, self.PW, self.A)
            _lib.check(nbytes, "rotate_bwd4_plan_bytes")
            if nbytes > 0:
                buf = torch.empty(int(nbytes), dtype=torch.uint8, device=self.device)
                with torch.cuda.device(self.device):
                    _lib.check(self._lib.ctpvae_rotate_bwd4_plan_build_f32(self.Tinv8.data_ptr(), self.A, self.H, self.W, self.PH,
                                                                           self.PW, self.py, self.px, buf.data_ptr(),
                                                                           _stream_ptr()), "rotate_bwd4_plan_build")
                self._bwd4_plan = buf
        return self._bwd4_plan

    def _build_exact_plan(self):
        self._want_exact_plan = False
        nbytes = self._lib.ctpvae_rotate_exact_plan_bytes(self.H, self.W, self.PH, self.PW, self.A)
        _lib.check(nbytes, "rotate_exact_plan_bytes")
        if nbytes == 0:
            return
        buf = torch.empty(int(nbytes), dtype=torch.uint8, device=self.device)
        with torch.cuda.device(self.device):
            _lib.check(self._lib.ctpvae_rotate_exact_plan_build_f32(self.T8.data_ptr(), self.Tinv8.data_ptr(), self.A, self.H,
                                                                    self.W, self.PH, self.PW, self.py, self.px, buf.data_ptr(),
                                                                    _stream_ptr()), "rotate_exact_plan_build")
            over = self._lib.ctpvae_rotate_exact_plan_overflowed(buf.data_ptr(), self.H, self.W, self.PH, self.PW, self.A,
                                                                 _stream_ptr())
        _lib.check(over, "rotate_exact_plan_overflowed")
        if over == 0:
            self._exact_plan = buf

    def _build_exact_bilinear_plan(self):
        nbytes = self._lib.ctpvae_rotate_exact_wplan_bytes(self.H, self.W, self.A)
        _lib.check(nbytes, "rotate_exact_wplan_bytes")
        buf = torch.empty(int(nbytes), dtype=torch.uint8, device=self.device)
        with torch.cuda.device(self.device):
            _lib.check(self._lib.ctpvae_rotate_exact_wplan_build_f32(
                self.T8.data_ptr(), self.Tinv8.data_ptr(), self.A, self.H, self.W, self.PH, self.PW, self.py, self.px,
                self.interp, buf.data_ptr(), _stream_ptr()), "rotate_exact_wplan_build")
            over = self._lib.ctpvae_rotate_exact_wplan_overflowed(buf.data_ptr(), self.H, self.W, self.A, _stream_ptr())
        _lib.check(over, "rotate_exact_wplan_overflowed")
        if over == 0:
            self._exact_bilin_plan = buf

    @property
    def planned(self):
        return self._fwd_plan is not None, self._want_bwd_plan

    @property
    def compact(self):
        return self._compact

    def dense_plan(self, S):
        if self._auto_dense_u16 and not (self.COMPACT_DENSE_WINDOW[0] <= S <= self.COMPACT_DENSE_WINDOW[1]):
            if self._u16_plan is None:
                self._u16_plan = self._build_plan(0)
            return self._u16_plan, False
        return self._fwd_plan, self._compact

    def forward_kernel_name(self, S):
        if self.fast:
            return "rotate_fwd_bilin_kernel<FAST>"
        if self._fwd_plan is None:
            return "rotate_fwd_fast_kernel"
        return "rotate_fwd_compact_kernel" if self.dense_plan(S)[1] else "rotate_fwd_planned_kernel"

    def forward_form(self, S, img=None):
        if self.forward_kernel_name(S) != "rotate_fwd_planned_kernel":
            return 0
        aligned = 1 if img is None or img.data_ptr() % 16 == 0 else 0
        return _lib.check(self._lib.ctpvae_rotate_fwd_planned_form(S, self.H, self.W, self.PH, self.PW, self.A, aligned),
                          "rotate_fwd_planned_form")

    def _run_compact(self, img_ptr, S, out_ptr, angles_i=None, n=0, mask=None, meas=None, dense=0, pnm=None, eps=0.0,
                     lp_ptr=None, dlp_ptr=None, part_ptr=None, sum_ptr=None, noise=0):
        if noise:
            return self._lib.ctpvae_rotate_fwd_compact_noise_f32(
                img_ptr, S, self.H, self.W, self.PH, self.PW, self.A, self._fwd_plan.data_ptr(),
                angles_i.data_ptr() if angles_i is not None else None, n,
                1 if (angles_i is not None and angles_i.device.type == "cpu") else 0, mask.data_ptr() if mask is not None else None,
                meas.data_ptr() if meas is not None else None, dense, pnm.data_ptr() if pnm is not None else None,
                ctypes.c_float(eps), noise, out_ptr, lp_ptr, dlp_ptr, part_ptr, sum_ptr, _stream_ptr(self._dev_index))
        return self._lib.ctpvae_rotate_fwd_compact_f32(
            img_ptr, S, self.H, self.W, self.PH, self.PW, self.A, self._fwd_plan.data_ptr(),
            angles_i.data_ptr() if angles_i is not None else None, n,
            1 if (angles_i is not None and angles_i.device.type == "cpu") else 0, mask.data_ptr() if mask is not None else None,
            meas.data_ptr() if meas is not None else None, dense, pnm.data_ptr() if pnm is not None else None,
            ctypes.c_float(eps), out_ptr, lp_ptr, dlp_ptr, part_ptr, sum_ptr, _stream_ptr(self._dev_index))

    def poisson_fused(self, n_sel=None):
        return self._compact and self.interp == _lib.NEAREST and (n_sel is None or 1 <= n_sel <= self.MAX_SEL)

    def _noise_code(self, noise, angles_i):
        if noise not in _lib.NOISE:
            raise ValueError(f"noise must be 'gaussian' or 'poisson' (got {noise!r})")
        code = _lib.NOISE[noise]
        if code and not self.poisson_fused(None if angles_i is None else angles_i.numel()):
            raise ValueError("noise='poisson' is fused into the step-coded (compact) plan's launch only (see poisson_fused): project, "
                             "then call poisson_log_prob on this geometry")
        return code

    def forward_loglik_sums(self, img, mask, meas, pnm, eps, angles_i=None, dense_inputs=False, with_dlp=True, noise="gaussian"):
        if self.interp != _lib.NEAREST:
            raise ValueError("forward_loglik needs a planned or tiled forward (nearest)")
        noise = self._noise_code(noise, angles_i)
        if angles_i is not None and not self.sel_supported(angles_i.numel()):
            if dense_inputs:
                idx = self._sel_dev(angles_i).long()
                mask, meas = mask.index_select(1, idx).contiguous(), meas.index_select(1, idx).contiguous()
            return self.subset(angles_i).forward_loglik_sums(img, mask, meas, pnm, eps, with_dlp=with_dlp)
        with torch.cuda.device(self._dev_index):
            S = img.shape[0]
            sums = _new_output((S,), torch.float32, self._tdev)
            ws = self._tile_workspace(S) if angles_i is None else None
            if ws is not None:
                self._check(img, (self.H, self.W), "img")
                self._check(meas, (self.A, self.PW), "meas")
                self._check(mask, (self.A,), "mask")
                if meas.shape[0] != S or mask.shape[0] != S or pnm.numel() != 1 or pnm.dtype != torch.float32 or pnm.device != img.device:
                    raise ValueError("mask [S][A], meas [S][A][PW] and a one-element float32 pnm on the same device are needed")
                dlp = _new_output((S, self.A, self.PW), torch.float32, self._tdev) if with_dlp else None
                part = self._part_workspace(S, self.A, 1)
                rc = self._lib.ctpvae_rotate_fwd_tiled_compact_f32(
                    img.data_ptr(), S, self.H, self.W, self.PH, self.PW, self.py, self.px, self.T8.data_ptr(), self.A,
                    self._tplan.data_ptr() if self._tplan is not None else None, ws.data_ptr(), mask.data_ptr(), meas.data_ptr(),
                    pnm.data_ptr(), ctypes.c_float(eps), None, None, dlp.data_ptr() if dlp is not None else None,
                    part.data_ptr(), sums.data_ptr(), _stream_ptr(self._dev_index))
                if rc:
                    _lib.check(rc, "rotate_fwd_tiled_compact")
                return sums, dlp
            if not self._compact:
                res = self._forward_loglik(img, mask, meas, pnm, eps, with_dlp=with_dlp, angles_i=angles_i,
                                           dense_inputs=dense_inputs)
                lp = res[1]
                partition = 0 if self._fwd_plan is not None else 1
                _lib.check(self._lib.ctpvae_loglik_object_sums_f32(lp.data_ptr(), S, lp.shape[1], self.PW, partition,
                                                                   sums.data_ptr(), _stream_ptr(self._dev_index)),
                           "loglik_object_sums")
                return sums, (res[2] if with_dlp else None)
            self._check(img, (self.H, self.W), "img")
            n = self.A if angles_i is None else self._check_sel(angles_i)
            n_in = self.A if (angles_i is None or dense_inputs) else n
            self._check(meas, (n_in, self.PW), "meas")
            self._check(mask, (n_in,), "mask")
            if meas.shape[0] != S or mask.shape[0] != S or pnm.numel() != 1 or pnm.dtype != torch.float32 or pnm.device != img.device:
                raise ValueError("mask [S][A], meas [S][A][PW] and a one-element float32 pnm on the same device are needed")
            dlp = _new_output((S, n, self.PW), torch.float32, self._tdev) if with_dlp else None
            part = self._part_workspace(S, n, 0)
            rc = self._run_compact(img.data_ptr(), S, None, angles_i, n if angles_i is not None else 0, mask, meas,
                                   1 if dense_inputs else 0, pnm, eps, None, dlp.data_ptr() if dlp is not None else None,
                                   part.data_ptr(), sums.data_ptr(), noise=noise)
            if rc:
                _lib.check(rc, "rotate_fwd_compact")
            return sums, dlp

# ... 676 lines not shown
```

include/ctpvae_radon.h:

```cpp
#ifndef CTPVAE_RADON_H
#define CTPVAE_RADON_H

#ifdef __cplusplus
extern "C" {
#endif

#define CTPVAE_OK 0
#define CTPVAE_EINVAL (-1)
#define CTPVAE_EHIP (-2)
#define CTPVAE_ENODEV (-3)

#define CTPVAE_NOISE_GAUSSIAN 0
#define CTPVAE_NOISE_POISSON 1
#define CTPVAE_NEAREST 0
#define CTPVAE_BILINEAR 1

#define CTPVAE_BWD_TF_COMPAT 0
#define CTPVAE_BWD_EXACT 1

typedef void *ctpvae_stream_t;

#define CTPVAE_ABI_VERSION 3400
int ctpvae_abi_version(void);
const char *ctpvae_last_error(void);
int ctpvae_device_count(void);
int ctpvae_tune_set(const char *name, int value);
int ctpvae_tune_active(void);

int ctpvae_num_proj_pix(int nx, int ny);
int ctpvae_pad_amounts(int n, int P, int *lo, int *hi);

int ctpvae_rotate_transforms_f32(const float *theta_dev, int A, int H, int W, float *T8_dev,
                                 float *Tinv8_dev, ctpvae_stream_t stream);
int ctpvae_rotate_transforms_host_f32(const float *theta, int A, int H, int W, float *T8, float *Tinv8);

int ctpvae_rotate_fwd_f32(const float *img_dev, int S, int H, int W, int PH, int PW, int py, int px,
                          const float *T8_dev, int A, int interp, float *sino_dev,
                          ctpvae_stream_t stream);

int ctpvae_rotate_fwd_f64(const double *img_dev, int S, int H, int W, int PH, int PW, int py, int px,
                          const float *T8_dev, int A, int interp, double *sino_dev, ctpvae_stream_t stream);
int ctpvae_rotate_bwd_f64(const double *gsino_dev, int S, int A, int PH, int PW, const float *T8_dev, int interp, int mode,
                          int H, int W, int py, int px, double *gimg_dev, ctpvae_stream_t stream);

int ctpvae_rotate_tile_shape(int H, int W, int interp, int *tile_h, int *tile_w);
long long ctpvae_rotate_fwd_tiled_workspace_bytes(int S, int H, int W, int PH, int PW, int A, int interp);
int ctpvae_rotate_fwd_tiled_f32(const float *img_dev, int S, int H, int W, int PH, int PW, int py, int px,
                                const float *T8_dev, int A, void *workspace_dev, float *sino_dev,
                                ctpvae_stream_t stream);

int ctpvae_rotate_fwd_tiled_interp_f32(const float *img_dev, int S, int H, int W, int PH, int PW, int py, int px,
                                       const float *T8_dev, int A, int interp, void *workspace_dev, float *sino_dev,
                                       ctpvae_stream_t stream);

int ctpvae_rotate_fwd_fast_f32(const float *img_dev, int S, int H, int W, int PH, int PW, int py, int px,
                               const float *T8_dev, int A, float *sino_dev, ctpvae_stream_t stream);
int ctpvae_rotate_fwd_tiled_fast_f32(const float *img_dev, int S, int H, int W, int PH, int PW, int py, int px,
                                     const float *T8_dev, int A, void *workspace_dev, float *sino_dev,
                                     ctpvae_stream_t stream);

int ctpvae_rotate_fwd_tiled_loglik_f32(const float *img_dev, int S, int H, int W, int PH, int PW, int py, int px,
                                       const float *T8_dev, int A, void *workspace_dev, const float *mask_dev,
                                       const float *meas_dev, const float *pnm_dev, float eps, float *sino_dev,
                                       float *lp_dev, float *dlp_dev, ctpvae_stream_t stream);

long long ctpvae_rotate_tplan_bytes(int H, int W, int PH, int PW, int A);
int ctpvae_rotate_tplan_build_f32(const float *T8_dev, int A, int H, int W, int PH, int PW, int py, int px, void *tplan_dev,
                                  ctpvae_stream_t stream);
int ctpvae_rotate_tplan_overflowed(const void *tplan_dev, int H, int W, int PH, int PW, int A, ctpvae_stream_t stream);
int ctpvae_rotate_fwd_tiled_compact_f32(const float *img_dev, int S, int H, int W, int PH, int PW, int py, int px,
                                        const float *T8_dev, int A, const void *tplan_dev, void *workspace_dev,
                                        const float *mask_dev, const float *meas_dev, const float *pnm_dev, float eps,
                                        float *sino_dev, float *lp_dev, float *dlp_dev, float *lp_part_dev, float *lp_sum_dev,
                                        ctpvae_stream_t stream);

int ctpvae_rotate_bwd_f32(const float *gsino_dev, int S, int A, int PH, int PW, const float *T8_dev,
                          int interp, int mode, int H, int W, int py, int px, float *gimg_dev,
                          ctpvae_stream_t stream);
int ctpvae_rotate_bwd_scaled_f32(const float *gsino_dev, int S, int A, int PH, int PW, const float *T8_dev,
                                 int interp, int mode, int H, int W, int py, int px, const float *scale_dev,
                                 long long scale_stride, float *gimg_dev, ctpvae_stream_t stream);

int ctpvae_rotate_plan_supported(int H, int W, int PH, int PW, int A, int interp, int which);
long long ctpvae_rotate_plan_bytes(int H, int W, int PH, int PW, int A, int which);
int ctpvae_rotate_plan_build_f32(const float *T8_dev, const float *Tinv8_dev, int A, int H, int W, int PH, int PW,
                                 int py, int px, void *fwd_plan_dev, void *bwd_plan_dev, ctpvae_stream_t stream);
int ctpvae_rotate_fwd_planned_f32(const float *img_dev, int S, int H, int W, int PH, int PW, int A,
                                  const void *fwd_plan_dev, float *sino_dev, ctpvae_stream_t stream);
int ctpvae_rotate_fwd_planned_form(int S, int H, int W, int PH, int PW, int A, int img_aligned16);
int ctpvae_rotate_fwd_planned_loglik_f32(const float *img_dev, int S, int H, int W, int PH, int PW, int A,
                                         const void *fwd_plan_dev, const float *mask_dev, const float *meas_dev,
                                         const float *pnm_dev, float eps, float *sino_dev, float *lp_dev,
                                         float *dlp_dev, ctpvae_stream_t stream);
int ctpvae_rotate_fwd_planned_sel_f32(const float *img_dev, int S, int H, int W, int PH, int PW, int A,
                                      const void *fwd_plan_dev, const int *angle_idx_dev, int n_idx, float *sino_dev,
                                      ctpvae_stream_t stream);
int ctpvae_rotate_fwd_planned_loglik_sel_f32(const float *img_dev, int S, int H, int W, int PH, int PW, int A,
                                             const void *fwd_plan_dev, const int *angle_idx_dev, int n_idx,
                                             const float *mask_dev, const float *meas_dev, int dense_inputs,
                                             const float *pnm_dev, float eps, float *sino_dev, float *lp_dev,
                                             float *dlp_dev, ctpvae_stream_t stream);
int ctpvae_rotate_cplan_supported(int H, int W, int PH, int PW, int A, int interp);
long long ctpvae_rotate_cplan_bytes(int H, int W, int PH, int PW, int A);
int ctpvae_rotate_cplan_build_f32(const float *T8_dev, int A, int H, int W, int PH, int PW, int py, int px, void *cplan_dev,
                                  ctpvae_stream_t stream);
int ctpvae_rotate_cplan_overflowed(const void *cplan_dev, int H, int W, int PH, int PW, int A, ctpvae_stream_t stream);
int ctpvae_rotate_fwd_compact_f32(const float *img_dev, int S, int H, int W, int PH, int PW, int A, const void *cplan_dev,
                                  const int *angle_idx, int n_idx, int idx_on_host, const float *mask_dev,
                                  const float *meas_dev, int dense_inputs, const float *pnm_dev, float eps, float *sino_dev,
                                  float *lp_dev, float *dlp_dev, float *lp_part_dev, float *lp_sum_dev, ctpvae_stream_t stream);
int ctpvae_rotate_fwd_compact_noise_f32(const float *img_dev, int S, int H, int W, int PH, int PW, int A, const void *cplan_dev,
                                        const int *angle_idx, int n_idx, int idx_on_host, const float *mask_dev,
                                        const float *meas_dev, int dense_inputs, const float *pnm_dev, float eps, int noise,
                                        float *sino_dev, float *lp_dev, float *dlp_dev, float *lp_part_dev, float *lp_sum_dev,
                                        ctpvae_stream_t stream);

int ctpvae_rotate_bwd_sel_scaled_f32(const float *gsino_dev, int S, int A_plan, int PH, int PW, const float *Tinv8_dev,
                                     const int *angle_idx_dev, int n_idx, int H, int W, int py, int px,
                                     const float *scale_dev, long long scale_stride, float *gimg_dev,
                                     ctpvae_stream_t stream);

long long ctpvae_rotate_bwd4_plan_bytes(int H, int W, int PH, int PW, int A);
int ctpvae_rotate_bwd4_plan_build_f32(const float *Tinv8_dev, int A, int H, int W, int PH, int PW, int py, int px,
                                      void *plan_dev, ctpvae_stream_t stream);
int ctpvae_rotate_bwd_planned_sel_scaled_f32(const float *gsino_dev, int S, int H, int W, int PH, int PW, int A,
                                             const void *bwd4_plan_dev, const int *angle_idx, int n_idx, int idx_on_host,
                                             const float *scale_dev, long long scale_stride, float *gimg_dev,
                                             ctpvae_stream_t stream);

long long ctpvae_rotate_bwd_step_plan_bytes(int H, int W, int A);
int ctpvae_rotate_bwd_step_plan_build_f32(const float *Tinv8_dev, int A, int H, int W, int PH, int PW, int py, int px, void *plan_dev,
                                          ctpvae_stream_t stream);
int ctpvae_rotate_bwd_step_plan_overflowed(const void *plan_dev, int H, int W, int A, ctpvae_stream_t stream);
int ctpvae_rotate_bwd_stepped_scaled_f32(const float *gsino_dev, int S, int A, int PH, int PW, const float *Tinv8_dev, int H, int W,
                                         int py, int px, const void *step_plan_dev, const float *scale_dev, long long scale_stride,
                                         float *gimg_dev, ctpvae_stream_t stream);

int ctpvae_rotate_bwd_planned_f32(const float *gsino_dev, int S, int H, int W, int PH, int PW, int A,
                                  const void *bwd_plan_dev, float *gimg_dev, ctpvae_stream_t stream);
int ctpvae_rotate_bwd_planned_scaled_f32(const float *gsino_dev, int S, int H, int W, int PH, int PW, int A,
                                         const void *bwd_plan_dev, const float *scale_dev, long long scale_stride,
                                         float *gimg_dev, ctpvae_stream_t stream);

long long ctpvae_rotate_exact_plan_bytes(int H, int W, int PH, int PW, int A);
int ctpvae_rotate_exact_plan_build_f32(const float *T8_dev, const float *Tinv8_dev, int A, int H, int W, int PH, int PW,
                                       int py, int px, void *plan_dev, ctpvae_stream_t stream);
int ctpvae_rotate_exact_plan_overflowed(const void *plan_dev, int H, int W, int PH, int PW, int A, ctpvae_stream_t stream);
int ctpvae_rotate_bwd_exact_planned_f32(const float *gsino_dev, int S, int H, int W, int PH, int PW, int A,
                                        const void *exact_plan_dev, float *gimg_dev, ctpvae_stream_t stream);

long long ctpvae_rotate_exact_wplan_bytes(int H, int W, int A);
int ctpvae_rotate_exact_wplan_build_f32(const float *T8_dev, const float *Tinv8_dev, int A, int H, int W, int PH, int PW,
                                        int py, int px, int interp, void *plan_dev, ctpvae_stream_t stream);
int ctpvae_rotate_exact_wplan_overflowed(const void *plan_dev, int H, int W, int A, ctpvae_stream_t stream);
int ctpvae_rotate_bwd_exact_wplan_f32(const float *gsino_dev, int S, int A, int PH, int PW, const float *Tinv8_dev,
                                      int H, int W, int py, int px, const void *plan_dev, float *gimg_dev,
                                      ctpvae_stream_t stream);

int ctpvae_siddon_dx(int ox, int oz, int pad);
int ctpvae_siddon_tables_f32(const float *theta, int dt, float *sin_out, float *cos_out, int *quadrant_out);
int ctpvae_siddon_fwd_f32(const float *obj_dev, int oy, int ox, int oz, const float *sin_dev,
                          const float *cos_dev, const int *quad_dev, int dt, int dx, float center,
                          float *data_dev, ctpvae_stream_t stream);

long long ctpvae_siddon_bwd_workspace_bytes(int oy, int ox, int oz, int dt, int dx);
int ctpvae_siddon_bwd_prepare_f32(int ox, int oz, const float *sin_dev, const float *cos_dev, const int *quad_dev, int dt, int dx,
                                  float center, void *workspace_dev, ctpvae_stream_t stream);
int ctpvae_siddon_bwd_prepared_f32(const float *data_dev, int oy, int ox, int oz, const float *sin_dev, const float *cos_dev,
                                   const int *quad_dev, int dt, int dx, float center, const void *workspace_dev,
                                   const float *colsum_dev, float *recon_dev, ctpvae_stream_t stream);
int ctpvae_siddon_bwd_f32(const float *data_dev, int oy, int ox, int oz, const float *sin_dev, const float *cos_dev,
                          const int *quad_dev, int dt, int dx, float center, void *workspace_dev, float *recon_dev,
// ... 159 lines not shown
```

Baseline: 109.8 million projections/s.

## Stage only touched image blocks in forward rotate via per-task footprint masks

Adds a plan section that records, for each angle/column-block task, a bitmask of the 4x32 image blocks its taps touch. A device-side DP then partitions tasks into contiguous groups that minimise a modelled cost, falling back to interleaved grouping. A masked forward kernel stages into LDS only the blocks in each group's union mask rather than the whole image. This is meant to cut global reads and LDS staging per workgroup, at the cost of extra plan-building kernels, a larger plan and a host sync to resolve the mode.

```diff
diff --git a/ct_pvae_amd/_lib.py b/ct_pvae_amd/_lib.py
--- a/ct_pvae_amd/_lib.py
+++ b/ct_pvae_amd/_lib.py
@@ -76,6 +76,11 @@
                                               _vp]),
     "ctpvae_rotate_fwd_planned_f32": (_c_int, [_vp, _c_int, _c_int, _c_int, _c_int, _c_int, _c_int, _vp, _vp, _vp]),
     "ctpvae_rotate_fwd_planned_form": (_c_int, [_c_int, _c_int, _c_int, _c_int, _c_int, _c_int, _c_int]),
+    "ctpvae_rotate_fwd_plan_section": (ctypes.c_longlong, [_c_int, _c_int, _c_int, _c_int, _c_int, _c_int, _c_int, _c_int]),
+    "ctpvae_fwd_group_table_ints": (_c_int, [_c_int, _c_int]),
+    "ctpvae_fwd_group_partition": (_c_int, [_vp, _vp, _c_int, _c_int, _vp]),
+    "ctpvae_rotate_fwd_planned_staging": (_c_int, [_c_int, _c_int, _c_int, _c_int, _c_int, _c_int, _vp, _c_int,
+                                                   ctypes.POINTER(ctypes.c_longlong), _vp]),
     "ctpvae_rotate_fwd_planned_loglik_f32": (_c_int, [_vp, _c_int, _c_int, _c_int, _c_int, _c_int, _c_int, _vp, _vp, _vp, _vp,
                                                       _c_float, _vp, _vp, _vp, _vp]),
     "ctpvae_rotate_bwd_planned_f32": (_c_int, [_vp, _c_int, _c_int, _c_int, _c_int, _c_int, _c_int, _vp, _vp, _vp]),
diff --git a/ct_pvae_amd/csrc/common.h b/ct_pvae_amd/csrc/common.h
--- a/ct_pvae_amd/csrc/common.h
+++ b/ct_pvae_amd/csrc/common.h
@@ -90,7 +90,7 @@
 enum Knob {
     kKnobNoPlan, kKnobForceGeneric, kKnobNs, kKnobG, kKnobWaves, kKnobBns, kKnobBw, kKnobSegNs, kKnobSegChunk,
     kKnobSegPpt, kKnobTiledNs, kKnobTiledG, kKnobSiddonNs, kKnobSiddonThreads, kKnobSiddonPpb, kKnobMaxSlices,
-    kKnobSiddonBwdNs, kKnobSiddonBwdChunks, kKnobNoCompact, kKnobSkew0, kKnobTiledSort, kKnobTiledPair, kKnobAffine, kKnobFakeStaticLds, kKnobFoldSums, kKnobTiledXcd, kKnobTiledWaves, kKnobTiledTh, kKnobReduceWaves, kKnobStepNs, kKnobStepLdsKb, kKnobTiledForce, kKnobBsort, kKnobMixG, kKnobMixG2, kKnobMixU1, kKnobNoMagic, kKnobMixG1, kKnobMixG3, kKnobMixU2, kKnobBrsplit, kKnobFwdFew, kKnobWtStores, kKnobBwdTail, kKnobCount
+    kKnobSiddonBwdNs, kKnobSiddonBwdChunks, kKnobNoCompact, kKnobSkew0, kKnobTiledSort, kKnobTiledPair, kKnobAffine, kKnobFakeStaticLds, kKnobFoldSums, kKnobTiledXcd, kKnobTiledWaves, kKnobTiledTh, kKnobReduceWaves, kKnobStepNs, kKnobStepLdsKb, kKnobTiledForce, kKnobBsort, kKnobMixG, kKnobMixG2, kKnobMixU1, kKnobNoMagic, kKnobMixG1, kKnobMixG3, kKnobMixU2, kKnobBrsplit, kKnobFwdFew, kKnobWtStores, kKnobBwdTail, kKnobFwdMask, kKnobCount
 };
 int knob(Knob k);
 
diff --git a/ct_pvae_amd/csrc/core.hip b/ct_pvae_amd/csrc/core.hip
--- a/ct_pvae_amd/csrc/core.hip
+++ b/ct_pvae_amd/csrc/core.hip
@@ -22,7 +22,7 @@
 
 static const char *const kKnobNames[kKnobCount] = {
     "NO_PLAN", "FORCE_GENERIC", "NS", "G", "WAVES", "BNS", "BW", "SEG_NS", "SEG_CHUNK", "SEG_PPT", "TILED_NS", "TILED_G",
-    "SIDDON_NS", "SIDDON_THREADS", "SIDDON_PPB", "MAX_SLICES", "SIDDON_BWD_NS", "SIDDON_BWD_CHUNKS", "NO_COMPACT", "SKEW0", "TILED_SORT", "TILED_PAIR", "AFFINE", "FAKE_STATIC_LDS", "FOLD_SUMS", "TILED_XCD", "TILED_WAVES", "TILED_TH", "REDUCE_WAVES", "STEP_NS", "STEP_LDS_KB", "TILED_FORCE", "BSORT", "MIXG", "MIXG_G2", "MIXG_U1", "NO_MAGIC", "MIXG_G1", "MIXG_G3", "MIXG_U2", "BRSPLIT", "FWD_FEW", "WT_STORES", "BWD_TAIL"};
+    "SIDDON_NS", "SIDDON_THREADS", "SIDDON_PPB", "MAX_SLICES", "SIDDON_BWD_NS", "SIDDON_BWD_CHUNKS", "NO_COMPACT", "SKEW0", "TILED_SORT", "TILED_PAIR", "AFFINE", "FAKE_STATIC_LDS", "FOLD_SUMS", "TILED_XCD", "TILED_WAVES", "TILED_TH", "REDUCE_WAVES", "STEP_NS", "STEP_LDS_KB", "TILED_FORCE", "BSORT", "MIXG", "MIXG_G2", "MIXG_U1", "NO_MAGIC", "MIXG_G1", "MIXG_G3", "MIXG_U2", "BRSPLIT", "FWD_FEW", "WT_STORES", "BWD_TAIL", "FWD_MASK"};
 static std::atomic<int> g_knobs[kKnobCount];
 static int find_knob(const char *name)
 {
diff --git a/ct_pvae_amd/csrc/fwd_groups.h b/ct_pvae_amd/csrc/fwd_groups.h
--- /dev/null
+++ b/ct_pvae_amd/csrc/fwd_groups.h
@@ -0,0 +1,130 @@
+#pragma once
+#include <hip/hip_runtime.h>
+
+namespace ctpvae {
+
+constexpr int kFwdMaskBits = 128;
+constexpr int kFwdMaskWords = 4;
+constexpr int kFwdGroupMaxG = 12;
+constexpr int kFwdGroupMaxTasks = 128;
+constexpr int kFwdTabHdr = 8;
+constexpr int kFwdTabRec = 8;
+
+__host__ __device__ inline int fwd_group_entries_padded(int T) { return (T + 7) / 8 * 8; }
+__host__ __device__ inline int fwd_group_table_ints(int G, int T) { return kFwdTabHdr + kFwdTabRec * G + fwd_group_entries_padded(T); }
+__host__ __device__ inline int fwd_group_ws_ints(int T) { return 3 * (kFwdGroupMaxG + 1) * (T + 1); }
+
+__host__ __device__ inline int fwd_mask_popc(const unsigned *m)
+{
+    int n = 0;
+    for (int w = 0; w < kFwdMaskWords; ++w)
+        for (unsigned v = m[w]; v; v &= v - 1) ++n;
+    return n;
+}
+__host__ __device__ inline int fwd_group_cost(int n, int blocks, int longest)
+{
+    if (n == 0) return 0;
+    return 250 + (blocks * 1024 + 4096 * (n < 16 ? n : 16)) / 70 + 90 * longest * ((n + 15) / 16);
+}
+
+__host__ __device__ inline void fwd_group_dp(const int *ng, const unsigned *mask, int T, int *ws)
+{
+    const int LV = kFwdGroupMaxG + 1, W1 = T + 1;
+    int *bmax = ws, *bsum = ws + LV * W1, *cut = ws + 2 * LV * W1;
+    const int kInf = 0x7fffffff;
+    const int Ge = kFwdGroupMaxG < T ? kFwdGroupMaxG : T;
+    for (int l = 0; l <= Ge; ++l)
+        for (int j = 0; j <= T; ++j) bmax[l * W1 + j] = kInf, bsum[l * W1 + j] = kInf, cut[l * W1 + j] = 0;
+    bmax[0] = 0, bsum[0] = 0;
+    for (int i = 0; i < T; ++i) {
+        unsigned u[kFwdMaskWords] = {0u, 0u, 0u, 0u};
+        int longest = 0;
+        for (int j = i + 1; j <= T; ++j) {
+            for (int w = 0; w < kFwdMaskWords; ++w) u[w] |= mask[(j - 1) * kFwdMaskWords + w];
+            longest = ng[j - 1] > longest ? ng[j - 1] : longest;
+            const int c = fwd_group_cost(j - i, fwd_mask_popc(u), longest);
+            for (int l = 1; l <= Ge; ++l) {
+                const int pm = bmax[(l - 1) * W1 + i];
+                if (pm == kInf) continue;
+                const int nm = pm > c ? pm : c, nsum = bsum[(l - 1) * W1 + i] + c;
+                int &dm = bmax[l * W1 + j], &ds = bsum[l * W1 + j];
+                if (nm < dm || (nm == dm && nsum < ds)) dm = nm, ds = nsum, cut[l * W1 + j] = i;
+            }
+        }
+    }
+}
+__host__ __device__ inline void fwd_group_emit(const int *ng, const unsigned *mask, const int *code, int T, int G, const int *ws, int *out)
+{
+    const int LV = kFwdGroupMaxG + 1, W1 = T + 1;
+    const int *bmax = ws, *cut = ws + 2 * LV * W1;
+    const int kInf = 0x7fffffff;
+    const int Ge = G < T ? G : T;
+    int cost_il = 0;
+    for (int gi = 0; gi < G; ++gi) {
+        unsigned u[kFwdMaskWords] = {0u, 0u, 0u, 0u};
+        int n = 0, longest = 0;
+        for (int m = gi; m < T; m += G, ++n) {
+            for (int w = 0; w < kFwdMaskWords; ++w) u[w] |= mask[m * kFwdMaskWords + w];
+            longest = ng[m] > longest ? ng[m] : longest;
+        }
+        const int c = fwd_group_cost(n, fwd_mask_popc(u), longest);
+        cost_il = c > cost_il ? c : cost_il;
+    }
+    int lbest = 0, cost = T > 0 ? kInf : 0;
+    for (int l = 1; l <= Ge; ++l)
+        if (bmax[l * W1 + T] <= cost) cost = bmax[l * W1 + T], lbest = l;
+#ifdef CTPVAE_TUNE_GROUPS_INTERLEAVED
+    const int helps = 0;
+#else
+    const int helps = T > 0 && cost < cost_il ? 1 : 0;
+#endif
+    int *rec = out + kFwdTabHdr, *ent = out + kFwdTabHdr + kFwdTabRec * G;
+    for (int i = 0; i < kFwdTabRec * G; ++i) rec[i] = 0;
+    for (int i = 0; i < fwd_group_entries_padded(T); ++i) ent[i] = 0;
+    if (helps) {
+        int j = T;
+        for (int l = lbest; l >= 1; --l) {
+            const int i = cut[l * W1 + j];
+            rec[(l - 1) * kFwdTabRec + 0] = i, rec[(l - 1) * kFwdTabRec + 1] = j - i;
+            for (int m = i; m < j; ++m) ent[m] = m;
+            j = i;
+        }
+    } else {
+        int pos = 0;
+        for (int gi = 0; gi < G; ++gi) {
+            rec[gi * kFwdTabRec + 0] = pos;
+            for (int m = gi; m < T; m += G) ent[pos++] = m;
+            rec[gi * kFwdTabRec + 1] = pos - rec[gi * kFwdTabRec + 0];
+        }
+    }
+    int busiest = 0;
+    for (int gi = 0; gi < G; ++gi) {
+        int *r = rec + gi * kFwdTabRec, *e = ent + r[0];
+        const int n = r[1];
+        for (int a = 1; a < n; ++a) {
+            const int m = e[a];
+            int b = a;
+            for (; b > 0 && (ng[e[b - 1]] < ng[m] || (ng[e[b - 1]] == ng[m] && e[b - 1] > m)); --b) e[b] = e[b - 1];
+            e[b] = m;
+        }
+        unsigned u[kFwdMaskWords] = {0u, 0u, 0u, 0u};
+        for (int a = 0; a < n; ++a)
+            for (int w = 0; w < kFwdMaskWords; ++w) u[w] |= mask[e[a] * kFwdMaskWords + w];
+        r[2] = n > 0 ? ng[e[0]] : 0;
+        r[3] = fwd_mask_popc(u);
+        for (int w = 0; w < kFwdMaskWords; ++w) r[4 + w] = (int)u[w];
+        busiest = r[3] > busiest ? r[3] : busiest;
+    }
+    if (code)
+        for (int i = 0; i < T; ++i) ent[i] = code[ent[i]];
+    out[0] = helps, out[1] = busiest, out[2] = helps ? cost : cost_il, out[3] = cost_il;
+    out[4] = out[5] = out[6] = out[7] = 0;
+}
+
+__host__ __device__ inline void fwd_group_partition(const int *ng, const unsigned *mask, const int *code, int T, int G, int *ws, int *out)
+{
+    fwd_group_dp(ng, mask, T, ws);
+    fwd_group_emit(ng, mask, code, T, G, ws, out);
+}
+
+}
diff --git a/ct_pvae_amd/csrc/lds_stage.h b/ct_pvae_amd/csrc/lds_stage.h
--- a/ct_pvae_amd/csrc/lds_stage.h
+++ b/ct_pvae_amd/csrc/lds_stage.h
@@ -212,6 +212,62 @@
     else stage_unit_pow2_m<NS, NB, false>(lds, src, rows, cs, src_stride, pitch, lane, wave, nwaves, between);
 }
 
+template <int NS, int NB, bool MIRROR, bool POISON>
+__device__ __forceinline__ void stage_unit_pow2_masked(float *lds, const float *const (&src)[NS], int rows, int cs, int src_stride, int pitch,
+                                                       int lane, int wave, int nwaves, unsigned long long mask_lo, unsigned long long mask_hi)
+{
+    const int h = lane >> 5, k = (lane & 31) >> 3, m = lane & 7, cols = 64 << cs, nrq = rows >> 2;
+    const int lo_src = k * src_stride + (MIRROR ? -(32 * h + 4 * m) : 32 * h + 4 * m);
+    const int lo_dst = k * pitch + 32 * h + 4 * m;
+    float4 v[NB][NS];
+    unsigned bits[NB];
+#pragma unroll
+    for (int i = 0; i < NB; ++i) {
+        const int pp = wave + i * nwaves, rq = pp >> cs, pc = pp & ((1 << cs) - 1);
+        const unsigned long long word = pp < 32 ? mask_lo : mask_hi;
+        bits[i] = rq < nrq && pp < 64 ? (unsigned)(word >> (2 * (pp & 31))) & 3u : 0u;
+        if constexpr (POISON) {
+#pragma unroll
+            for (int n = 0; n < NS; ++n) v[i][n] = float4{__builtin_nanf(""), __builtin_nanf(""), __builtin_nanf(""), __builtin_nanf("")};
+        }
+        if (bits[i] == 0u) continue;
+        const int so = 4 * rq * src_stride + (MIRROR ? cols - 4 - 64 * pc : 64 * pc);
+        if ((bits[i] >> h) & 1u) {
+#pragma unroll
+            for (int n = 0; n < NS; ++n) v[i][n] = *reinterpret_cast<const float4 *>(src[n] + so + lo_src);
+        }
+    }
+#pragma unroll
+    for (int i = 0; i < NB; ++i) {
+        const int pp = wave + i * nwaves, rq = pp >> cs, pc = pp & ((1 << cs) - 1);
+        if (POISON ? (rq >= nrq || pp >= 64) : bits[i] == 0u) continue;
+        if (!POISON && !((bits[i] >> h) & 1u)) continue;
+        const int cell = 4 * rq * pitch + 64 * pc + lo_dst;
+        if constexpr (NS == 1) {
+            float *d = lds + cell;
+            d[0] = MIRROR ? v[i][0].w : v[i][0].x;
+            d[1] = MIRROR ? v[i][0].z : v[i][0].y;
+            d[2] = MIRROR ? v[i][0].y : v[i][0].z;
+            d[3] = MIRROR ? v[i][0].x : v[i][0].w;
+        } else {
+            typedef float vec_t __attribute__((ext_vector_type(NS)));
+            vec_t *d = reinterpret_cast<vec_t *>(lds) + cell;
+            vec_t w0, w1, w2, w3;
+#pragma unroll
+            for (int n = 0; n < NS; ++n) {
+                w0[n] = MIRROR ? v[i][n].w : v[i][n].x;
+                w1[n] = MIRROR ? v[i][n].z : v[i][n].y;
+                w2[n] = MIRROR ? v[i][n].y : v[i][n].z;
+                w3[n] = MIRROR ? v[i][n].x : v[i][n].w;
+            }
+            d[0] = w0;
+            d[1] = w1;
+            d[2] = w2;
+            d[3] = w3;
+        }
+    }
+}
+
 __host__ __device__ inline int contig_rows_units_per_quad(int cols) { return (cols + 15) >> 4; }
 __host__ __device__ inline unsigned contig_rows_magic(int cols) { return 65536u / (unsigned)contig_rows_units_per_quad(cols) + 1u; }
 __host__ __device__ inline int contig_rows_units(int rows, int cols) { return ((rows + 3) >> 2) * contig_rows_units_per_quad(cols); }
diff --git a/ct_pvae_amd/csrc/rotate_fwd_masked.h b/ct_pvae_amd/csrc/rotate_fwd_masked.h
--- /dev/null
+++ b/ct_pvae_amd/csrc/rotate_fwd_masked.h
@@ -0,0 +1,13 @@
+#pragma once
+#include "rotate_fwd_shared.h"
+
+namespace ctpvae {
+
+long long fwd_masked_plan_bytes(const PlanGeom &g, const FwdLayout &L);
+int fwd_masked_build(const PlanGeom &g, const FwdLayout &L, void *plan_dev, ctpvae_stream_t stream);
+int fwd_masked_resolve(const PlanGeom &g, const FwdLayout &L, const void *plan_dev, ctpvae_stream_t stream);
+int fwd_masked_mode(const PlanGeom &g, const FwdLayout &L, int G, const void *plan_dev, int *busiest_blocks);
+int fwd_masked_launch(int mode, int ns, unsigned grid, int waves, size_t shmem, ctpvae_stream_t stream, const float *img_dev, float *sino_dev,
+                      const FwdFewArgs &k, const PlanGeom &g, const FwdLayout &L, const void *plan_dev);
+
+}
diff --git a/ct_pvae_amd/csrc/rotate_fwd_masked.hip b/ct_pvae_amd/csrc/rotate_fwd_masked.hip
--- /dev/null
+++ b/ct_pvae_amd/csrc/rotate_fwd_masked.hip
@@ -0,0 +1,334 @@
+#include <atomic>
+#include <mutex>
+#include <unordered_map>
+#include <vector>
+
+#include "common.h"
+#include "fwd_groups.h"
+#include "lds_stage.h"
+#include "rotate_plan.h"
+#include "rotate_fwd_masked.h"
+#include "tune_stamps.h"
+
+namespace ctpvae {
+
+struct FwdMaskLayout {
+    int ok, T;
+    long long off_mask, off_tab, bytes;
+};
+static bool fwd_mask_ok(const PlanGeom &g, const FwdLayout &L)
+{
+    return !L.skew0 && (g.W == 64 || g.W == 128 || g.W == 256) && g.H % 4 == 0 && (g.H / 4) * (g.W / 64) <= kFwdMaskBits / 2 &&
+           (long long)g.A * L.nJB <= kFwdGroupMaxTasks;
+}
+static long long fwd_tab_offset_ints(int G, int c, int T)
+{
+    long long o = 0;
+    for (int x = 1; x < G; ++x) o += 2ll * ((fwd_group_table_ints(x, T) + 63) / 64 * 64);
+    return o + (long long)c * ((fwd_group_table_ints(G, T) + 63) / 64 * 64);
+}
+static FwdMaskLayout fwd_mask_layout(const PlanGeom &g, const FwdLayout &L)
+{
+    FwdMaskLayout M;
+    M.ok = fwd_mask_ok(g, L) ? 1 : 0;
+    M.T = g.A * L.nJB;
+    M.off_mask = M.off_tab = M.bytes = L.bytes;
+    if (M.ok) {
+        M.off_mask = (L.bytes + 255) / 256 * 256;
+        M.off_tab = (M.off_mask + (long long)M.T * kFwdMaskWords * 4 + 255) / 256 * 256;
+        M.bytes = M.off_tab + fwd_tab_offset_ints(kFwdGroupMaxG + 1, 0, M.T) * 4;
+    }
+    return M;
+}
+__global__ __launch_bounds__(64) void rotate_fwd_mask_kernel(PlanGeom g, FwdLayout L, const char *__restrict__ plan, unsigned *__restrict__ mask)
+{
+    const int a = blockIdx.y, jb = blockIdx.x, lane = threadIdx.x;
+    const int *rng = reinterpret_cast<const int *>(plan + L.off_rng);
+    const uint4 *idx = reinterpret_cast<const uint4 *>(plan + L.off_idx);
+    const int first = rng[(a * L.nJB + jb) * 2], last = kRngBias - rng[(a * L.nJB + jb) * 2 + 1];
+    const int cb = g.W / 32;
+    unsigned u[kFwdMaskWords] = {0u, 0u, 0u, 0u};
+    for (int gq = first; gq <= last; ++gq) {
+        const uint4 q = idx[((size_t)a * L.Galloc + gq) * L.PWpad + jb * 64 + lane];
+        const unsigned w[4] = {q.x, q.y, q.z, q.w};
+#pragma unroll
+        for (int e = 0; e < 8; ++e) {
+            const int tap = (int)((w[e >> 1] >> (16 * (e & 1))) & 0xffffu);
+            if (tap == L.zero) continue;
+            const int row = tap / L.pitch, col = tap - row * L.pitch;
+            const int bit = (row >> 2) * cb + (col >> 5);
+#pragma unroll
+            for (int x = 0; x < kFwdMaskWords; ++x)
+                if ((bit >> 5) == x) u[x] |= 1u << (bit & 31);
+        }
+    }
+#pragma unroll
+    for (int x = 0; x < kFwdMaskWords; ++x) {
+        for (int off = 32; off > 0; off >>= 1) u[x] |= __shfl_xor(u[x], off, 64);
+        if (lane == 0) mask[(a * L.nJB + jb) * kFwdMaskWords + x] = u[x];
+    }
+}
+__global__ __launch_bounds__(64) void rotate_fwd_groups_kernel(int A, FwdLayout L, FwdMaskLayout M, char *__restrict__ plan)
+{
+    __shared__ int ws[3 * (kFwdGroupMaxG + 1) * (kFwdGroupMaxTasks + 1)];
+    __shared__ int ng[kFwdGroupMaxTasks], code[kFwdGroupMaxTasks];
+    __shared__ unsigned tmask[kFwdGroupMaxTasks * kFwdMaskWords];
+    if (threadIdx.x != 0) return;
+    const int c = blockIdx.x;
+    const int *clist = reinterpret_cast<const int *>(plan + L.off_clist) + c * (A + 1);
+    const int *rng = reinterpret_cast<const int *>(plan + L.off_rng);
+    const unsigned *mask = reinterpret_cast<const unsigned *>(plan + M.off_mask);
+    const int ncls = clist[0], T = ncls * L.nJB;
+    for (int m = 0; m < T; ++m) {
+        const int jb = m / ncls, a = clist[1 + m - jb * ncls];
+        const int first = rng[(a * L.nJB + jb) * 2], last = kRngBias - rng[(a * L.nJB + jb) * 2 + 1];
+        ng[m] = last >= first ? last - first + 1 : 0;
+        code[m] = a | (jb << 16);
+        for (int x = 0; x < kFwdMaskWords; ++x) tmask[m * kFwdMaskWords + x] = mask[(a * L.nJB + jb) * kFwdMaskWords + x];
+    }
+    int *tab = reinterpret_cast<int *>(plan + M.off_tab);
+    fwd_group_dp(ng, tmask, T, ws);
+    for (int G = 1; G <= kFwdGroupMaxG; ++G) {
+        long long o = 0;
+        for (int x = 1; x < G; ++x) o += 2ll * ((fwd_group_table_ints(x, M.T) + 63) / 64 * 64);
+        o += (long long)c * ((fwd_group_table_ints(G, M.T) + 63) / 64 * 64);
+        fwd_group_emit(ng, tmask, code, T, G, ws, tab + o);
+    }
+}
+
+struct FwdMaskArgs {
+    const int *tab;
+    int cstride;
+};
+template <int NS, bool POISON>
+__global__ __launch_bounds__(1024) void rotate_fwd_planned_kernel_few_masked(const float *__restrict__ img, float *__restrict__ sino, FwdFewArgs k,
+                                                                             FwdMaskArgs mk)
+{
+    typedef typename SliceVec<NS>::type vec_t;
+    extern __shared__ float lds[];
+    const unsigned q = blockIdx.x, per8 = 8u * (unsigned)k.wgs;
+    const unsigned octet = div_by_magic(q >> 3, k.inv_wgs), rem = q - octet * per8;
+    int u, wg;
+    if ((int)(octet + 1) * 8 <= k.units) {
+        wg = rem >> 3;
+        u = octet * 8 + (rem & 7);
+    } else {
+        const unsigned ru = div_by_magic(rem, k.inv_wgs);
+        u = octet * 8 + ru;
+        wg = rem - ru * k.wgs;
+    }
+    const int s = u * NS;
+    const bool has2 = NS == 2 && s + 1 < k.S;
+    const int c = wg & 1, gi = wg >> 1;
+    const int lane = threadIdx.x & 63, nwaves = blockDim.x >> 6;
+    const int wave = __builtin_amdgcn_readfirstlane(threadIdx.x >> 6);
+    const float *im = img + (size_t)s * k.slice;
+    CTPVAE_PSTAMP(0);
+
+    const int *tabc = mk.tab + c * mk.cstride;
+    const int *rec = tabc + kFwdTabHdr + kFwdTabRec * gi;
+    const int ntask = rec[1];
+    const int *ent = tabc + kFwdTabHdr + kFwdTabRec * k.G + rec[0];
+    const unsigned long long mask_lo = (unsigned)rec[4] | ((unsigned long long)(unsigned)rec[5] << 32);
+    const unsigned long long mask_hi = (unsigned)rec[6] | ((unsigned long long)(unsigned)rec[7] << 32);
+#ifdef CTPVAE_TUNE_NOIDX
+    const size_t st = 0;
+#else
+    const size_t st = (size_t)k.st;
+#endif
+    struct Task {
+        bool valid;
+        int a, j, ng;
+        const uint4 *p;
+        uint4 q0, q1, q2, q3;
+    };
+    auto fill = [&](Task &t, int e) {
+        const int jb = e >> 16;
+        t.a = e & 0xffff;
+        const int first = k.rng[(t.a * k.nJB + jb) * 2], last = kRngBias - k.rng[(t.a * k.nJB + jb) * 2 + 1];
+        const int g0 = last >= first ? first : 0;
+        t.ng = last >= first ? last - first + 1 : 0;
+        t.j = lane_to_bin(k.PW, jb, lane);
+        t.p = k.idx + ((size_t)t.a * k.ast + (size_t)g0 * k.st + jb * 64) + lane;
+        t.q0 = t.p[0];
+        t.q1 = t.p[st];
+        t.q2 = t.p[2 * st];
+        t.q3 = t.p[3 * st];
+        t.p += 4 * st;
+    };
+    Task cur;
+    cur.valid = wave < ntask;
+    if (cur.valid) fill(cur, ent[wave]);
+    int *next_task = reinterpret_cast<int *>(lds + (k.zero + 1) * NS);
+    if (threadIdx.x == 0) *next_task = nwaves;
+
+    {
+        const float *srcs[NS];
+        srcs[0] = im;
+        if constexpr (NS == 2) srcs[1] = im + (has2 ? (size_t)k.slice : 0);
+        if (c == 0) stage_unit_pow2_masked<NS, 8 / NS, true, POISON>(lds, srcs, k.rows, k.cs, k.src_stride, k.pitch, lane, wave, nwaves, mask_lo, mask_hi);
+        else stage_unit_pow2_masked<NS, 8 / NS, false, POISON>(lds, srcs, k.rows, k.cs, k.src_stride, k.pitch, lane, wave, nwaves, mask_lo, mask_hi);
+    }
+    if (threadIdx.x < NS) lds[k.zero * NS + threadIdx.x] = 0.0f;
+    CTPVAE_PSTAMP(1);
+    __syncthreads();
+    CTPVAE_PSTAMP(2);
+
+    while (cur.valid) {
+        int m = 0;
+        if (lane == 0) m = atomicAdd(next_task, 1);
+        Task nxt;
+        {
+            const int mn = __builtin_amdgcn_readfirstlane(m);
+            nxt.valid = mn < ntask;
+            if (nxt.valid) fill(nxt, ent[mn]);
+        }
+        const int ng = __builtin_amdgcn_readfirstlane(cur.ng);
+        const uint4 *p = cur.p;
+        vec_t acc = 0.0f;
+        if (ng > 0) {
+            uint4 q0 = cur.q0, q1 = cur.q1, q2 = cur.q2, q3 = cur.q3;
+            vec_t va[8], vb[8];
+            gather8(lds, q0, va);
+            q0 = p[0];
+            CTPVAE_FWD_WALK_U16
+        }
+        if ((unsigned)cur.j < (unsigned)k.PW) {
+            const size_t o = ((size_t)s * k.A + cur.a) * k.PW + cur.j;
+            if constexpr (NS == 1) {
+                sino[o] = acc;
+            } else {
+                sino[o] = acc.x;
+                if (has2) sino[o + (size_t)k.A * k.PW] = acc.y;
+            }
+        }
+        cur = nxt;
+    }
+    CTPVAE_PSTAMP(3);
+}
+struct FwdMaskInfo {
+    int H, W, PH, PW, A;
+    int helps[kFwdGroupMaxG + 1][2], busiest[kFwdGroupMaxG + 1][2];
+};
+static std::mutex g_fwd_mask_mu;
+static std::unordered_map<const void *, FwdMaskInfo> g_fwd_mask_info;
+static void fwd_mask_forget(const void *plan)
+{
+    std::lock_guard<std::mutex> lock(g_fwd_mask_mu);
+    g_fwd_mask_info.erase(plan);
+}
+static bool fwd_mask_lookup(const void *plan, const PlanGeom &g, FwdMaskInfo &out)
+{
+    std::lock_guard<std::mutex> lock(g_fwd_mask_mu);
+    const auto it = g_fwd_mask_info.find(plan);
+    if (it == g_fwd_mask_info.end()) return false;
+    const FwdMaskInfo &f = it->second;
+    if (f.H != g.H || f.W != g.W || f.PH != g.PH || f.PW != g.PW || f.A != g.A) return false;
+    out = f;
+    return true;
+}
+
+constexpr bool kFwdMaskRule = false;
+int fwd_masked_mode(const PlanGeom &g, const FwdLayout &L, int G, const void *plan, int *busiest_blocks)
+{
+    if (busiest_blocks) *busiest_blocks = 0;
+    if (!fwd_mask_ok(g, L) || G < 1 || G > kFwdGroupMaxG) return 0;
+    const int v = knob(kKnobFwdMask);
+    if (v == 0) return 0;
+    FwdMaskInfo f;
+    const bool known = fwd_mask_lookup(plan, g, f);
+    if (known && busiest_blocks) *busiest_blocks = std::max(f.busiest[G][0], f.busiest[G][1]);
+    if (v == 1 || v == 2) return v;
+    return kFwdMaskRule && known && (f.helps[G][0] || f.helps[G][1]) ? 1 : 0;
+}
+
+
+long long fwd_masked_plan_bytes(const PlanGeom &g, const FwdLayout &L) { return fwd_mask_layout(g, L).bytes; }
+
+int fwd_masked_build(const PlanGeom &g, const FwdLayout &L, void *plan_dev, ctpvae_stream_t stream)
+{
+    fwd_mask_forget(plan_dev);
+    const FwdMaskLayout M = fwd_mask_layout(g, L);
+    if (M.ok) {
+        hipLaunchKernelGGL(rotate_fwd_mask_kernel, dim3(L.nJB, g.A), dim3(64), 0, (hipStream_t)stream, g, L, (const char *)plan_dev,
+                           reinterpret_cast<unsigned *>((char *)plan_dev + M.off_mask));
+        CTPVAE_LAUNCH_CHECK("rotate_fwd_mask_kernel");
+        hipLaunchKernelGGL(rotate_fwd_groups_kernel, dim3(2), dim3(64), 0, (hipStream_t)stream, g.A, L, M, (char *)plan_dev);
+        CTPVAE_LAUNCH_CHECK("rotate_fwd_groups_kernel");
+    }
+    return CTPVAE_OK;
+}
+
+int fwd_masked_resolve(const PlanGeom &g, const FwdLayout &L, const void *plan_dev, ctpvae_stream_t stream)
+{
+    const FwdMaskLayout M = fwd_mask_layout(g, L);
+    FwdMaskInfo f;
+    if (M.ok && !fwd_mask_lookup(plan_dev, g, f)) {
+        f = FwdMaskInfo{g.H, g.W, g.PH, g.PW, g.A, {}, {}};
+        int hdr[kFwdGroupMaxG + 1][2][kFwdTabHdr];
+        for (int G = 1; G <= kFwdGroupMaxG; ++G)
+            for (int c = 0; c < 2; ++c)
+                CTPVAE_HIP(hipMemcpyAsync(hdr[G][c], (const char *)plan_dev + M.off_tab + fwd_tab_offset_ints(G, c, M.T) * 4, sizeof(hdr[G][c]),
+                                          hipMemcpyDeviceToHost, (hipStream_t)stream));
+        CTPVAE_HIP(hipStreamSynchronize((hipStream_t)stream));
+        for (int G = 1; G <= kFwdGroupMaxG; ++G)
+            for (int c = 0; c < 2; ++c) f.helps[G][c] = hdr[G][c][0] != 0, f.busiest[G][c] = hdr[G][c][1];
+        std::lock_guard<std::mutex> lock(g_fwd_mask_mu);
+        g_fwd_mask_info[plan_dev] = f;
+    }
+    return CTPVAE_OK;
+}
+
+int fwd_masked_launch(int mode, int ns, unsigned grid, int waves, size_t shmem, ctpvae_stream_t stream, const float *img_dev, float *sino_dev,
+                      const FwdFewArgs &k, const PlanGeom &g, const FwdLayout &L, const void *plan_dev)
+{
+    const FwdMaskLayout M = fwd_mask_layout(g, L);
+    FwdMaskArgs mk;
+    mk.tab = reinterpret_cast<const int *>((const char *)plan_dev + M.off_tab) + fwd_tab_offset_ints(k.G, 0, M.T);
+    mk.cstride = (int)(fwd_tab_offset_ints(k.G, 1, M.T) - fwd_tab_offset_ints(k.G, 0, M.T));
+    auto launch_masked = [&](auto kernel) -> int {
+        static std::atomic<unsigned long long> attr_set{0}, abs_ok{0};
+        CTPVAE_REQUIRE_NO_STATIC_LDS(kernel, "rotate_fwd_planned_kernel_few_masked", abs_ok);
+        CTPVAE_SET_MAX_LDS_ONCE(kernel, attr_set);
+        hipLaunchKernelGGL(kernel, dim3(grid), dim3(64 * waves), shmem, (hipStream_t)stream, img_dev, sino_dev, k, mk);
+        CTPVAE_LAUNCH_CHECK("rotate_fwd_planned_kernel_few_masked");
+        return CTPVAE_OK;
+    };
+    if (mode == 2)
+        return ns == 2 ? launch_masked(rotate_fwd_planned_kernel_few_masked<2, true>) : launch_masked(rotate_fwd_planned_kernel_few_masked<1, true>);
+    return ns == 2 ? launch_masked(rotate_fwd_planned_kernel_few_masked<2, false>) : launch_masked(rotate_fwd_planned_kernel_few_masked<1, false>);
+}
+
+}
+
+using namespace ctpvae;
+
+extern "C" {
+
+int ctpvae_fwd_group_table_ints(int G, int T)
+{
+    CTPVAE_REQUIRE(G >= 1 && G <= kFwdGroupMaxG && T >= 0 && T <= kFwdGroupMaxTasks, "fwd_group_table_ints: 1 <= G <= %d, 0 <= T <= %d", kFwdGroupMaxG, kFwdGroupMaxTasks);
+    return fwd_group_table_ints(G, T);
+}
+
+int ctpvae_fwd_group_partition(const int *ng, const unsigned *masks, int T, int G, int *table_out)
+{
+    CTPVAE_REQUIRE(ng && masks && table_out, "fwd_group_partition: null pointer");
+    CTPVAE_REQUIRE(G >= 1 && G <= kFwdGroupMaxG && T >= 0 && T <= kFwdGroupMaxTasks, "fwd_group_partition: 1 <= G <= %d, 0 <= T <= %d", kFwdGroupMaxG, kFwdGroupMaxTasks);
+    std::vector<int> ws((size_t)fwd_group_ws_ints(T));
+    fwd_group_partition(ng, masks, nullptr, T, G, ws.data(), table_out);
+    return fwd_group_table_ints(G, T);
+}
+
+long long ctpvae_rotate_fwd_plan_section(int H, int W, int PH, int PW, int A, int what, int G, int cls)
+{
+    if (H <= 0 || W <= 0 || PH < H || PW < W || A <= 0) return fail(CTPVAE_EINVAL, "rotate_fwd_plan_section: bad sizes");
+    const PlanGeom g{H, W, PH, PW, 0, 0, A};
+    const FwdMaskLayout M = fwd_mask_layout(g, fwd_layout(g));
+    if (!M.ok) return 0;
+    if (what == 0) return M.off_mask;
+    CTPVAE_REQUIRE(what == 1 && G >= 1 && G <= kFwdGroupMaxG && (cls == 0 || cls == 1), "rotate_fwd_plan_section: what = 0 (masks) or 1 (the table of 1 <= G <= %d, class 0 / 1)", kFwdGroupMaxG);
+    return M.off_tab + fwd_tab_offset_ints(G, cls, M.T) * 4;
+}
+
+}
diff --git a/ct_pvae_amd/csrc/rotate_fwd_shared.h b/ct_pvae_amd/csrc/rotate_fwd_shared.h
--- /dev/null
+++ b/ct_pvae_amd/csrc/rotate_fwd_shared.h
@@ -0,0 +1,134 @@
+#pragma once
+#include <algorithm>
+
+#include "common.h"
+#include "rotate_plan.h"
+
+namespace ctpvae {
+
+struct FwdLayout {
+    int nJB, PWpad, NG, Galloc, pitch, zero, skew0;
+    long long off_cls, off_clist, off_first, off_rng, off_idx, bytes;
+};
+
+inline FwdLayout fwd_layout(const PlanGeom &g)
+{
+    FwdLayout L;
+    L.nJB = num_bin_blocks(g.PW);
+    L.PWpad = L.nJB * 64;
+    L.NG = ceil_div(g.PH, 8);
+    L.Galloc = L.NG + 8;
+    L.skew0 = knob(kKnobSkew0) > 0 ? 1 : 0;
+    L.pitch = L.skew0 ? (g.W + 31) / 32 * 32 : pitch_mod32_is_1(g.W);
+    if (L.skew0) L.Galloc += 6;
+    L.zero = g.H * L.pitch;
+    L.off_cls = 0;
+    L.off_clist = (long long)g.A * 4;
+    L.off_first = (L.off_clist + 2ll * (g.A + 1) * 4 + 8 + 255) / 256 * 256;
+    L.off_rng = (L.off_first + (long long)g.A * L.PWpad * 4 + 255) / 256 * 256;
+    L.off_idx = (L.off_rng + (long long)g.A * L.nJB * 8 + 255) / 256 * 256;
+    L.bytes = L.off_idx + (long long)g.A * L.Galloc * L.PWpad * 16;
+    return L;
+}
+
+constexpr int kRngBias = 0x7f7f7f7f;
+
+__device__ __forceinline__ void unpack2(unsigned pk, int &lo4, int &hi4)
+{
+    asm("v_lshlrev_b32_sdwa %0, 2, %1 dst_sel:DWORD dst_unused:UNUSED_PAD src0_sel:DWORD src1_sel:WORD_0"
+        : "=v"(lo4)
+        : "v"(pk));
+    asm("v_lshlrev_b32_sdwa %0, 2, %1 dst_sel:DWORD dst_unused:UNUSED_PAD src0_sel:DWORD src1_sel:WORD_1"
+        : "=v"(hi4)
+        : "v"(pk));
+}
+__device__ __forceinline__ float lds_at(const float *, int byte_off) { return *(lds_cptr)(size_t)(unsigned)byte_off; }
+__device__ __forceinline__ void unpack2x8(unsigned pk, int &lo8, int &hi8)
+{
+    asm("v_lshlrev_b32_sdwa %0, 3, %1 dst_sel:DWORD dst_unused:UNUSED_PAD src0_sel:DWORD src1_sel:WORD_0"
+        : "=v"(lo8)
+        : "v"(pk));
+    asm("v_lshlrev_b32_sdwa %0, 3, %1 dst_sel:DWORD dst_unused:UNUSED_PAD src0_sel:DWORD src1_sel:WORD_1"
+        : "=v"(hi8)
+        : "v"(pk));
+}
+__device__ __forceinline__ void gather8(const float *lds, const uint4 q, f32x2 (&v)[8])
+{
+    int a[8];
+    unpack2x8(q.x, a[0], a[1]);
+    unpack2x8(q.y, a[2], a[3]);
+    unpack2x8(q.z, a[4], a[5]);
+    unpack2x8(q.w, a[6], a[7]);
+#pragma unroll
+    for (int e = 0; e < 8; ++e) v[e] = *(const __attribute__((address_space(3))) f32x2 *)(size_t)(unsigned)a[e];
+}
+__device__ __forceinline__ void gather8(const float *lds, const uint4 q, float (&v)[8])
+{
+    int a0, a1, a2, a3, a4, a5, a6, a7;
+    unpack2(q.x, a0, a1);
+    unpack2(q.y, a2, a3);
+    unpack2(q.z, a4, a5);
+    unpack2(q.w, a6, a7);
+    v[0] = lds_at(lds, a0);
+    v[1] = lds_at(lds, a1);
+    v[2] = lds_at(lds, a2);
+    v[3] = lds_at(lds, a3);
+    v[4] = lds_at(lds, a4);
+    v[5] = lds_at(lds, a5);
+    v[6] = lds_at(lds, a6);
+    v[7] = lds_at(lds, a7);
+}
+
+__host__ __device__ inline unsigned div_magic(unsigned d) { return d > 1 ? (unsigned)((1ull << 32) / d) + 1u : 0u; }
+__host__ __device__ inline unsigned div_by_magic(unsigned x, unsigned magic) { return magic ? (unsigned)(((unsigned long long)x * magic) >> 32) : x; }
+__host__ __device__ inline unsigned div_magic_floor(unsigned d) { return d > 1 ? (unsigned)((1ull << 32) / d) : 0xffffffffu; }
+__host__ __device__ inline unsigned div_by_magic_floor(unsigned x, unsigned magic, unsigned d)
+{
+    const unsigned q = (unsigned)(((unsigned long long)x * magic) >> 32);
+    return q + (x - q * d >= d ? 1u : 0u);
+}
+
+
+#define CTPVAE_PADD(VC) _Pragma("unroll") for (int e = 0; e < 8; ++e) acc += VC[e];
+#define CTPVAE_PSTEP(QN, VN, VC, LOADNEXT)    \
+                gather8(lds, QN, VN);                                                              \
+                LOADNEXT;                                                                          \
+                __builtin_amdgcn_sched_barrier(0);                                                 \
+                CTPVAE_PADD(VC)
+#define CTPVAE_FWD_WALK_U16                                                                        \
+            int n = 0;                                                                             \
+            for (; n + 4 < ng; n += 4) {    \
+                CTPVAE_PSTEP(q1, vb, va, q1 = p[st])                             \
+                CTPVAE_PSTEP(q2, va, vb, q2 = p[2 * st])                          \
+                CTPVAE_PSTEP(q3, vb, va, q3 = p[3 * st])                          \
+                CTPVAE_PSTEP(q0, va, vb, (p += 4 * st, q0 = p[0]))                \
+            }                                                                                      \
+            if (n + 1 >= ng) {    \
+                CTPVAE_PADD(va)                                                                    \
+            } else {                                                                               \
+                CTPVAE_PSTEP(q1, vb, va, (void)0)                                                  \
+                if (n + 2 >= ng) {                                                                 \
+                    CTPVAE_PADD(vb)                                                                \
+                } else {                                                                           \
+                    CTPVAE_PSTEP(q2, va, vb, (void)0)                                              \
+                    if (n + 3 >= ng) {                                                             \
+                        CTPVAE_PADD(va)                                                            \
+                    } else {                                                                       \
+                        CTPVAE_PSTEP(q3, vb, va, (void)0)                                          \
+                        CTPVAE_PADD(vb)                                                            \
+                    }                                                                              \
+                }                                                                                  \
+            }
+
+struct FwdFewArgs {
+    const int *clist;
+    const unsigned *inv_ncls;
+    const int *rng;
+    const uint4 *idx;
+    int A, A1, rows, cs, src_stride, pitch, zero, PW, nJB;
+    int st, ast;
+    int G, wgs, S, units, slice;
+    unsigned inv_wgs;
+};
+
+}
diff --git a/ct_pvae_amd/csrc/rotate_plan.hip b/ct_pvae_amd/csrc/rotate_plan.hip
--- a/ct_pvae_amd/csrc/rotate_plan.hip
+++ b/ct_pvae_amd/csrc/rotate_plan.hip
@@ -4,18 +4,17 @@
 #include <cstdlib>
 #include <type_traits>
 
+
 #include "common.h"
 #include "lds_stage.h"
 #include "loglik_math.h"
 #include "rotate_plan.h"
+#include "rotate_fwd_shared.h"
+#include "rotate_fwd_masked.h"
 #include "tune_stamps.h"
 
 namespace ctpvae {
 
-struct FwdLayout {
-    int nJB, PWpad, NG, Galloc, pitch, zero, skew0;
-    long long off_cls, off_clist, off_first, off_rng, off_idx, bytes;
-};
 constexpr int kBwdPitch = 257;
 constexpr int kBwdChunk = 64;
 struct BwdLayout {
@@ -23,25 +22,6 @@
     long long bytes;
 };
 
-static FwdLayout fwd_layout(const PlanGeom &g)
-{
-    FwdLayout L;
-    L.nJB = num_bin_blocks(g.PW);
-    L.PWpad = L.nJB * 64;
-    L.NG = ceil_div(g.PH, 8);
-    L.Galloc = L.NG + 8;
-    L.skew0 = knob(kKnobSkew0) > 0 ? 1 : 0;
-    L.pitch = L.skew0 ? (g.W + 31) / 32 * 32 : pitch_mod32_is_1(g.W);
-    if (L.skew0) L.Galloc += 6;
-    L.zero = g.H * L.pitch;
-    L.off_cls = 0;
-    L.off_clist = (long long)g.A * 4;
-    L.off_first = (L.off_clist + 2ll * (g.A + 1) * 4 + 8 + 255) / 256 * 256;
-    L.off_rng = (L.off_first + (long long)g.A * L.PWpad * 4 + 255) / 256 * 256;
-    L.off_idx = (L.off_rng + (long long)g.A * L.nJB * 8 + 255) / 256 * 256;
-    L.bytes = L.off_idx + (long long)g.A * L.Galloc * L.PWpad * 16;
-    return L;
-}
 static int bwd_tail_dwords(int A, int dup)
 {
     const int r = A % 16;
@@ -123,7 +103,6 @@
     }
     first[(size_t)a * L.PWpad + jb * 64 + lane] = f;
 }
-constexpr int kRngBias = 0x7f7f7f7f;
 __global__ __launch_bounds__(64) void rotate_fwd_plan_kernel(PlanGeom g, const float *__restrict__ T8, FwdLayout L,
                                                              char *__restrict__ plan)
 {
@@ -224,61 +203,6 @@
     cell[1] = (unsigned char)hit1;
 }
 
-__device__ __forceinline__ void unpack2(unsigned pk, int &lo4, int &hi4)
-{
-    asm("v_lshlrev_b32_sdwa %0, 2, %1 dst_sel:DWORD dst_unused:UNUSED_PAD src0_sel:DWORD src1_sel:WORD_0"
-        : "=v"(lo4)
-        : "v"(pk));
-    asm("v_lshlrev_b32_sdwa %0, 2, %1 dst_sel:DWORD dst_unused:UNUSED_PAD src0_sel:DWORD src1_sel:WORD_1"
-        : "=v"(hi4)
-        : "v"(pk));
-}
-__device__ __forceinline__ float lds_at(const float *, int byte_off) { return *(lds_cptr)(size_t)(unsigned)byte_off; }
-__device__ __forceinline__ void unpack2x8(unsigned pk, int &lo8, int &hi8)
-{
-    asm("v_lshlrev_b32_sdwa %0, 3, %1 dst_sel:DWORD dst_unused:UNUSED_PAD src0_sel:DWORD src1_sel:WORD_0"
-        : "=v"(lo8)
-        : "v"(pk));
-    asm("v_lshlrev_b32_sdwa %0, 3, %1 dst_sel:DWORD dst_unused:UNUSED_PAD src0_sel:DWORD src1_sel:WORD_1"
-        : "=v"(hi8)
-        : "v"(pk));
-}
-__device__ __forceinline__ void gather8(const float *lds, const uint4 q, f32x2 (&v)[8])
-{
-    int a[8];
-    unpack2x8(q.x, a[0], a[1]);
-    unpack2x8(q.y, a[2], a[3]);
-    unpack2x8(q.z, a[4], a[5]);
-    unpack2x8(q.w, a[6], a[7]);
-#pragma unroll
-    for (int e = 0; e < 8; ++e) v[e] = *(const __attribute__((address_space(3))) f32x2 *)(size_t)(unsigned)a[e];
-}
-__device__ __forceinline__ void gather8(const float *lds, const uint4 q, float (&v)[8])
-{
-    int a0, a1, a2, a3, a4, a5, a6, a7;
-    unpack2(q.x, a0, a1);
-    unpack2(q.y, a2, a3);
-    unpack2(q.z, a4, a5);
-    unpack2(q.w, a6, a7);
-    v[0] = lds_at(lds, a0);
-    v[1] = lds_at(lds, a1);
-    v[2] = lds_at(lds, a2);
-    v[3] = lds_at(lds, a3);
-    v[4] = lds_at(lds, a4);
-    v[5] = lds_at(lds, a5);
-    v[6] = lds_at(lds, a6);
-    v[7] = lds_at(lds, a7);
-}
-
-__host__ __device__ inline unsigned div_magic(unsigned d) { return d > 1 ? (unsigned)((1ull << 32) / d) + 1u : 0u; }
-__host__ __device__ inline unsigned div_by_magic(unsigned x, unsigned magic) { return magic ? (unsigned)(((unsigned long long)x * magic) >> 32) : x; }
-__host__ __device__ inline unsigned div_magic_floor(unsigned d) { return d > 1 ? (unsigned)((1ull << 32) / d) : 0xffffffffu; }
-__host__ __device__ inline unsigned div_by_magic_floor(unsigned x, unsigned magic, unsigned d)
-{
-    const unsigned q = (unsigned)(((unsigned long long)x * magic) >> 32);
-    return q + (x - q * d >= d ? 1u : 0u);
-}
-
 __global__ __launch_bounds__(64) void rotate_class_list_kernel(int A, FwdLayout L, char *__restrict__ plan)
 {
     const int *cls = reinterpret_cast<const int *>(plan + L.off_cls);
@@ -301,36 +225,6 @@
 }
 
 constexpr int kSelRounds = 4;
-#define CTPVAE_PADD(VC) _Pragma("unroll") for (int e = 0; e < 8; ++e) acc += VC[e];
-#define CTPVAE_PSTEP(QN, VN, VC, LOADNEXT)    \
-                gather8(lds, QN, VN);                                                              \
-                LOADNEXT;                                                                          \
-                __builtin_amdgcn_sched_barrier(0);                                                 \
-                CTPVAE_PADD(VC)
-#define CTPVAE_FWD_WALK_U16                                                                        \
-            int n = 0;                                                                             \
-            for (; n + 4 < ng; n += 4) {    \
-                CTPVAE_PSTEP(q1, vb, va, q1 = p[st])                             \
-                CTPVAE_PSTEP(q2, va, vb, q2 = p[2 * st])                          \
-                CTPVAE_PSTEP(q3, vb, va, q3 = p[3 * st])                          \
-                CTPVAE_PSTEP(q0, va, vb, (p += 4 * st, q0 = p[0]))                \
-            }                                                                                      \
-            if (n + 1 >= ng) {    \
-                CTPVAE_PADD(va)                                                                    \
-            } else {                                                                               \
-                CTPVAE_PSTEP(q1, vb, va, (void)0)                                                  \
-                if (n + 2 >= ng) {                                                                 \
-                    CTPVAE_PADD(vb)                                                                \
-                } else {                                                                           \
-                    CTPVAE_PSTEP(q2, va, vb, (void)0)                                              \
-                    if (n + 3 >= ng) {                                                             \
-                        CTPVAE_PADD(va)                                                            \
-                    } else {                                                                       \
-                        CTPVAE_PSTEP(q3, vb, va, (void)0)                                          \
-                        CTPVAE_PADD(vb)                                                            \
-                    }                                                                              \
-                }                                                                                  \
-            }
 template <int NS, bool EPI, bool SEL>
 __global__ __launch_bounds__(1024) void rotate_fwd_planned_kernel(const float *__restrict__ img, PlanGeom g, FwdLayout L,
                                                                   const char *__restrict__ plan, int wgs_per_slice,
@@ -529,16 +423,6 @@
     CTPVAE_PSTAMP(3);
 }
 
-struct FwdFewArgs {
-    const int *clist;
-    const unsigned *inv_ncls;
-    const int *rng;
-    const uint4 *idx;
-    int A, A1, rows, cs, src_stride, pitch, zero, PW, nJB;
-    int st, ast;
-    int G, wgs, S, units, slice;
-    unsigned inv_wgs;
-};
 template <int NS>
 __global__ __launch_bounds__(1024) void rotate_fwd_planned_kernel_few(const float *__restrict__ img, float *__restrict__ sino, FwdFewArgs k)
 {
@@ -642,6 +526,7 @@
     }
     CTPVAE_PSTAMP(3);
 }
+
 #undef CTPVAE_FWD_WALK_U16
 #undef CTPVAE_PSTEP
 #undef CTPVAE_PADD
@@ -855,7 +740,7 @@
 {
     if (H <= 0 || W <= 0 || PH < H || PW < W || A <= 0) return fail(CTPVAE_EINVAL, "rotate_plan_bytes: bad sizes");
     const PlanGeom g{H, W, PH, PW, 0, 0, A};
-    return which == 0 ? fwd_layout(g).bytes : bwd_layout(g).bytes;
+    return which == 0 ? fwd_masked_plan_bytes(g, fwd_layout(g)) : bwd_layout(g).bytes;
 }
 
 int ctpvae_rotate_plan_build_f32(const float *T8_dev, const float *Tinv8_dev, int A, int H, int W, int PH, int PW, int py,
@@ -879,6 +764,7 @@
         CTPVAE_LAUNCH_CHECK("rotate_fwd_plan_kernel");
         hipLaunchKernelGGL(rotate_class_list_kernel, dim3(1), dim3(64), 0, (hipStream_t)stream, A, L, (char *)fwd_plan_dev);
         CTPVAE_LAUNCH_CHECK("rotate_class_list_kernel");
+        if (int rc = fwd_masked_build(g, L, fwd_plan_dev, stream)) return rc;
     }
     if (bwd_plan_dev) {
         CTPVAE_REQUIRE(Tinv8_dev, "rotate_plan_build: backward plan needs the inverted transforms");
@@ -1120,6 +1006,8 @@
         k.PW = PW, k.nJB = L.nJB, k.st = L.PWpad, k.ast = L.Galloc * L.PWpad;
         k.G = sh.wgs_per_slice / 2, k.wgs = sh.wgs_per_slice, k.S = S, k.units = sh.units, k.slice = H * W;
         k.inv_wgs = div_magic((unsigned)sh.wgs_per_slice);
+        if (const int mode = fwd_masked_mode(g, L, k.G, fwd_plan_dev, nullptr))
+            return fwd_masked_launch(mode, ns, (unsigned)sh.grid, sh.waves, sh.shmem, stream, img_dev, sino_dev, k, g, L, fwd_plan_dev);
         auto launch_few = [&](auto kernel) -> int {
             static std::atomic<unsigned long long> attr_set{0}, abs_ok{0};
             CTPVAE_REQUIRE_NO_STATIC_LDS(kernel, "rotate_fwd_planned_kernel_few", abs_ok);
@@ -1153,6 +1041,22 @@
     FwdShape sh;
     if (int rc = fwd_planned_shape(S, H, W, PH, PW, A, false, 0, sh)) return rc;
     return fwd_few_ok(sh, true, img_aligned16 != 0) ? 1 : 0;
+}
+
+int ctpvae_rotate_fwd_planned_staging(int S, int H, int W, int PH, int PW, int A, const void *fwd_plan_dev, int img_aligned16,
+                                      long long *bytes_out, ctpvae_stream_t stream)
+{
+    CTPVAE_REQUIRE(fwd_plan_dev, "rotate_fwd_planned_staging: null pointer");
+    FwdShape sh;
+    if (int rc = fwd_planned_shape(S, H, W, PH, PW, A, false, 0, sh)) return rc;
+    if (int rc = fwd_masked_resolve(sh.g, sh.L, fwd_plan_dev, stream)) return rc;
+    const long long whole = (long long)H * W * 4 * sh.ns;
+    if (bytes_out) *bytes_out = whole;
+    if (!fwd_few_ok(sh, true, img_aligned16 != 0)) return 0;
+    int blocks = 0;
+    const int mode = fwd_masked_mode(sh.g, sh.L, sh.wgs_per_slice / 2, fwd_plan_dev, &blocks);
+    if (mode && bytes_out) *bytes_out = (long long)blocks * 512 * sh.ns;
+    return mode;
 }
 
 int ctpvae_rotate_fwd_planned_f32(const float *img_dev, int S, int H, int W, int PH, int PW, int A, const void *fwd_plan_dev,
diff --git a/ct_pvae_amd/forward_functions.py b/ct_pvae_amd/forward_functions.py
--- a/ct_pvae_amd/forward_functions.py
+++ b/ct_pvae_amd/forward_functions.py
@@ -216,6 +216,9 @@
                 self.T8.data_ptr(), self.Tinv8.data_ptr(), self.A, self.H, self.W, self.PH, self.PW, self.py, self.px,
                 buf.data_ptr() if which == 0 else None, buf.data_ptr() if which == 1 else None, _stream_ptr()),
                 "rotate_plan_build")
+            if which == 0 and not torch.cuda.is_current_stream_capturing():
+                _lib.check(self._lib.ctpvae_rotate_fwd_planned_staging(1, self.H, self.W, self.PH, self.PW, self.A, buf.data_ptr(), 1,
+                                                                       None, _stream_ptr()), "rotate_fwd_planned_staging")
         return buf
 
     def _build_compact_plan(self):
@@ -316,6 +319,34 @@
         aligned = 1 if img is None or img.data_ptr() % 16 == 0 else 0
         return _lib.check(self._lib.ctpvae_rotate_fwd_planned_form(S, self.H, self.W, self.PH, self.PW, self.A, aligned),
                           "rotate_fwd_planned_form")
+
+    def forward_staging(self, S, img=None):
+        if self.forward_kernel_name(S) != "rotate_fwd_planned_kernel":
+            return 0, 0
+        aligned = 1 if img is None or img.data_ptr() % 16 == 0 else 0
+        nbytes = ctypes.c_longlong(0)
+        with torch.cuda.device(self.device):
+            mode = _lib.check(self._lib.ctpvae_rotate_fwd_planned_staging(
+                S, self.H, self.W, self.PH, self.PW, self.A, self.dense_plan(S)[0].data_ptr(), aligned, ctypes.byref(nbytes),
+                _stream_ptr()), "rotate_fwd_planned_staging")
+        return mode, int(nbytes.value)
+
+    def forward_plan_sections(self):
+        plan = self._u16_plan if self._u16_plan is not None else (None if self._compact else self._fwd_plan)
+        geo = (self.H, self.W, self.PH, self.PW, self.A)
+        off = self._lib.ctpvae_rotate_fwd_plan_section(*geo, 0, 0, 0) if plan is not None else 0
+        if off <= 0:
+            return None
+        nJB = (self.PW - (self.PW >> 1) + 31) // 32
+        host = plan.cpu().numpy()
+        masks = host[off: off + self.A * nJB * 16].view("uint32").reshape(self.A, nJB, 4).copy()
+        tables = {}
+        for G in range(1, 13):
+            n = _lib.check(self._lib.ctpvae_fwd_group_table_ints(G, self.A * nJB), "fwd_group_table_ints")
+            for c in (0, 1):
+                o = self._lib.ctpvae_rotate_fwd_plan_section(*geo, 1, G, c)
+                tables[G, c] = host[o: o + 4 * n].view("int32").copy()
+        return masks, tables
 
     def _run_compact(self, img_ptr, S, out_ptr, angles_i=None, n=0, mask=None, meas=None, dense=0, pnm=None, eps=0.0,
                      lp_ptr=None, dlp_ptr=None, part_ptr=None, sum_ptr=None, noise=0):
diff --git a/include/ctpvae_radon.h b/include/ctpvae_radon.h
--- a/include/ctpvae_radon.h
+++ b/include/ctpvae_radon.h
@@ -88,6 +88,11 @@
 int ctpvae_rotate_fwd_planned_f32(const float *img_dev, int S, int H, int W, int PH, int PW, int A,
                                   const void *fwd_plan_dev, float *sino_dev, ctpvae_stream_t stream);
 int ctpvae_rotate_fwd_planned_form(int S, int H, int W, int PH, int PW, int A, int img_aligned16);
+long long ctpvae_rotate_fwd_plan_section(int H, int W, int PH, int PW, int A, int what, int G, int cls);
+int ctpvae_fwd_group_table_ints(int G, int T);
+int ctpvae_fwd_group_partition(const int *ng, const unsigned *masks, int T, int G, int *table_out);
+int ctpvae_rotate_fwd_planned_staging(int S, int H, int W, int PH, int PW, int A, const void *fwd_plan_dev, int img_aligned16,
+                                      long long *bytes_out, ctpvae_stream_t stream);
 int ctpvae_rotate_fwd_planned_loglik_f32(const float *img_dev, int S, int H, int W, int PH, int PW, int A,
                                          const void *fwd_plan_dev, const float *mask_dev, const float *meas_dev,
                                          const float *pnm_dev, float eps, float *sino_dev, float *lp_dev,
```

Measured after the change: 109.7 million projections/s (median of 2 runs). Within noise of the previous version (-0.0%).
